# agsiddhant/PBML_Mantle_Convection

Measured on AMD Instinct MI355X. Metric: training samples/sec (2-D 506x506 Stokes fields), higher is better.
Workload: dtype f16+bf16; 1 GPU; CFG-3: symmetric U-Net (levels 5, c_h 16, k 5, repeats 3, reflect) + L1 data loss + divergence + Stokes momentum residual, 506x506, per-GPU batch 32, Adam, HIP-graph replay; global_batch=32, parallelism=dp1

## Files before the change

### include/mantle_hip.h

```cpp
#ifndef MANTLE_HIP_H
#define MANTLE_HIP_H

#include <stddef.h>
#include <stdint.h>

#ifdef __cplusplus
extern "C" {
#endif

#define MC_OK 0
#define MC_EINVAL (-1)
#define MC_EUNSUPPORTED (-2)
#define MC_EWORKSPACE (-3)

enum { MC_F32 = 0, MC_BF16 = 1, MC_MIX16 = 2 };
enum { MC_PAD_ZEROS = 0, MC_PAD_REPLICATE = 1, MC_PAD_REFLECT = 2 };
enum { MC_ACT_NONE = 0, MC_ACT_GELU = 1, MC_ACT_RELU = 2, MC_ACT_SILU = 3, MC_ACT_TANH = 4,
       MC_ACT_SELU = 5, MC_ACT_ELU = 6 };
enum { MC_POST_NONE = 0,
       MC_POST_ACT = 1,
       MC_POST_GN_ACT = 2   };
enum { MC_GSRC_NONE = 0,
       MC_GSRC_PLAIN = 1,
       MC_GSRC_PADFOLD = 2,
       MC_GSRC_PADFOLD_POOL = 3,
       MC_GSRC_PLAIN_POOL = 4   };

typedef struct {
  int32_t n;
  int32_t h, w;
  int32_t c_in0;
  int32_t c_in1;
  int32_t c_out;
  int32_t k;
  int32_t pad;
  int32_t pad_mode;
  int32_t dtype;
  int32_t sym_h;
  int32_t c_out_split;
  int32_t out_f32;
  int32_t sym_v;
  int32_t sym_hv;
} mc_conv_desc;

typedef struct {
  const void* ptr;
  int32_t kind;
  int32_t pad;
  int32_t pad_mode;
  int32_t pool;
  int32_t hs, ws;
  int32_t c8_total;
  int32_t cb_off;
} mc_grad_src;

typedef struct {
  const float* coef0;
  const float* coef1;
  int32_t act0, act1;
} mc_conv_prologue;

typedef struct {
  const void* y;
  const float* coef;
  int32_t act;
  int32_t pad;
  int32_t pad_mode;
  int32_t hs, ws;
  float* partials;
  int32_t part_stride;
  int32_t y_f16;
} mc_conv_epilogue;

int mc_version(void);
const char* mc_strerror(int code);

int mc_pack_nchw(const float* x, int32_t n, int32_t c, int32_t src_c, int32_t h, int32_t w, int32_t pad_w,
                 int32_t pad_mode, const float* chan_scale, int32_t dtype, void* out, void* stream);
int mc_unpack_nchw(const void* x, int32_t n, int32_t c, int32_t h, int32_t w, int32_t crop_w,
                   const float* mean_nc, int32_t dtype, float* out, void* stream);
int mc_pack_grad_nchw(const float* g, int32_t n, int32_t c, int32_t h, int32_t w, int32_t crop_w,
                      const float* mean_nc, int32_t dtype, void* out, void* stream);
int mc_sum_hw(const float* x, int32_t nc, int32_t hw, float scale, float* out, void* stream);

size_t mc_packed_weight_bytes(const mc_conv_desc* d, int32_t dgrad);
int mc_pack_weights(const mc_conv_desc* d, const float* w_unique, int32_t dgrad, void* packed,
                    void* stream);
const char* mc_conv_kernel_name(const mc_conv_desc* d);
int32_t mc_conv_tiles(const mc_conv_desc* d);
int mc_conv2d(const mc_conv_desc* d, const void* x0, const void* x1, const void* packed_w,
              const float* bias, void* y0, void* y1, float* stat_partials, void* stream);
int mc_conv2d_fused(const mc_conv_desc* d, const void* x0, const void* x1, const mc_conv_prologue* pro,
                    const void* packed_w, const float* bias, void* y0, void* y1, float* stat_partials,
                    const mc_conv_epilogue* epi, void* stream);
size_t mc_wgrad_partial_bytes(const mc_conv_desc* d);
size_t mc_conv_bank_read_extent(const mc_conv_desc* d);
int mc_conv2d_wgrad(const mc_conv_desc* d, const void* x0, const void* x1, const void* dy,
                    void* partials, void* stream);
int mc_conv2d_wgrad_finalize(const mc_conv_desc* d, const void* partials, float* dw_unique,
                             float* dbias, void* stream);
int mc_conv2d_wgrad_fused(const mc_conv_desc* d, const void* x0, const void* x1, const mc_conv_prologue* pro,
                          const void* dy, void* partials, void* stream);
int mc_pack_weights_batched(const mc_conv_desc* descs, const float* const* w_unique, const int32_t* dgrad,
                            void* const* packed, int32_t n, void* stream);
int mc_conv2d_wgrad_finalize_batched(const mc_conv_desc* descs, const void* const* partials, float* const* dw_unique,
                                     float* const* dbias, int32_t n, void* stream);

int mc_fold_padded(void* buf, int32_t n, int32_t c, int32_t hs, int32_t ws, int32_t pad, int32_t pad_mode,
                   int32_t dtype, void* stream);
int mc_fold_padded2(void* buf0, int32_t c0, void* buf1, int32_t c1, int32_t n, int32_t hs, int32_t ws, int32_t pad, int32_t pad_mode,
                    int32_t dtype, void* stream);
int32_t mc_fold_blocks(int32_t hs, int32_t ws, int32_t pad, int32_t pad_mode);
int mc_fold_padded_dz(void* buf, int32_t n, int32_t c, int32_t hs, int32_t ws, int32_t pad, int32_t pad_mode,
                      int32_t dtype, const void* y, const float* coef, int32_t act, float* partials,
                      int32_t part_stride_blocks, int32_t part_first_block, void* stream);

int mc_gn_partials(const void* y, int32_t n, int32_t c, int32_t h, int32_t w, int32_t dtype, int32_t tiles, float* part,
                   void* stream);
int mc_gn_finalize(const float* stat_partials, int32_t n, int32_t tiles, int32_t c, int32_t groups,
                   int32_t hw, float eps, float* stats_ng2, float* chan_mean, void* stream);
int mc_gn_finalize_coef(const float* stat_partials, int32_t n, int32_t tiles, int32_t c, int32_t groups, int32_t hw,
                        float eps, const float* gamma, const float* beta, float* stats_ng2, float* coef4, void* stream);

int mc_gn_act_fwd(const void* y, int32_t n, int32_t c, int32_t h, int32_t w, int32_t groups,
                  const float* stats_ng2, const float* gamma, const float* beta, int32_t post,
                  int32_t act, int32_t pool, int32_t dtype, void* a, void* pooled, void* stream);
int mc_gn_act_fwd_small(const void* y, const float* stat_partials, int32_t tiles, int32_t n, int32_t c, int32_t h, int32_t w,
                        int32_t groups, float eps, const float* gamma, const float* beta, int32_t act, int32_t pool,
                        int32_t dtype, float* stats_ng2, void* a, void* pooled, void* stream);
int32_t mc_gn_bwd_blocks(int32_t h, int32_t w);
int mc_gn_act_bwd_reduce(const void* y, int32_t n, int32_t c, int32_t h, int32_t w, int32_t groups,
                         const float* stats_ng2, const float* gamma, const float* beta, int32_t post,
                         int32_t act, int32_t dtype, const mc_grad_src* g0, const mc_grad_src* g1,
                         float* partials, void* stream);
int mc_gn_act_bwd_finalize(const float* partials, int32_t n, int32_t blocks, int32_t c, int32_t groups,
                           int32_t hw, const float* gamma, float* m12_ng2, float* dgamma, float* dbeta,
                           void* stream);
int mc_gn_act_bwd_finalize_n(const float* partials, int32_t n, int32_t blocks, int32_t c, int32_t groups, int32_t hw,
                             const float* gamma, float* m12_ng2, float* chan_sums, void* stream);
int mc_gn_act_bwd_apply(const void* y, int32_t n, int32_t c, int32_t h, int32_t w, int32_t groups,
                        const float* stats_ng2, const float* m12_ng2, const float* gamma,
                        const float* beta, int32_t post, int32_t act, int32_t dtype,
                        const mc_grad_src* g0, const mc_grad_src* g1, void* dy, void* stream);
int mc_gn_act_bwd_small(const void* y, int32_t n, int32_t c, int32_t h, int32_t w, int32_t groups, const float* stats_ng2,
                        const float* gamma, const float* beta, int32_t act, int32_t dtype, const mc_grad_src* g0,
                        const mc_grad_src* g1, void* dy, float* chan_sums, void* stream);
int mc_gn_param_grads_batched(const float* const* chan_sums, const int32_t* n, const int32_t* c, float* const* dgamma,
                              float* const* dbeta, int32_t jobs, void* stream);
int mc_gn_bwd_apply_dz(const mc_grad_src* dz, const void* y, int32_t n, int32_t c, int32_t h, int32_t w, int32_t groups,
                       const float* coef, const float* m12_ng2, int32_t dtype, void* dy, void* stream);
int mc_concat_cb8(const void* const* srcs, const int32_t* src_c, int32_t n_src, int32_t n, int32_t h, int32_t w,
                  int32_t dtype, void* out, void* stream);
int mc_cat_grad_gather(const mc_grad_src* g, int32_t c_total, int32_t c_off, int32_t c, int32_t n, int32_t h, int32_t w,
                       int32_t dtype, void* out, void* stream);
int mc_gsrc_sum(const mc_grad_src* g0, const mc_grad_src* g1, int32_t n, int32_t c, int32_t h, int32_t w,
                int32_t dtype, void* out, void* stream);

int mc_rect_copy(const void* src, int32_t hs, int32_t ws, int32_t sy, int32_t sx, void* dst, int32_t hd, int32_t wd,
                 int32_t dy, int32_t dx, int32_t rh, int32_t rw, int32_t n, int32_t c, int32_t accumulate, int32_t dtype,
                 void* stream);

int mc_avgpool_fwd(const void* x, int32_t n, int32_t c, int32_t h, int32_t w, int32_t f, int32_t dtype,
                   void* out, void* stream);
int mc_bicubic_fwd(const void* x, int32_t n, int32_t c, int32_t hi, int32_t wi, int32_t ho, int32_t wo,
                   const int32_t* idx_y, const float* wgt_y, const int32_t* idx_x, const float* wgt_x,
                   int32_t dtype, void* out, void* stream);
int mc_bicubic_fwd_act(const void* x, const float* coef, int32_t act, int32_t n, int32_t c, int32_t hi, int32_t wi,
                       int32_t ho, int32_t wo, const int32_t* idx_y, const float* wgt_y, const int32_t* idx_x,
                       const float* wgt_x, int32_t dtype, void* out, void* stream);
int mc_bicubic_bwd(const mc_grad_src* g, int32_t n, int32_t c, int32_t hi, int32_t wi, int32_t ho, int32_t wo,
                   const int32_t* ty_start, const int32_t* ty_j, const float* ty_w,
                   const int32_t* tx_start, const int32_t* tx_j, const float* tx_w,
                   int32_t dtype, void* dx, void* stream);
int mc_bicubic_bwd_taps(const mc_grad_src* gs, int32_t n, int32_t c, int32_t hi, int32_t wi, int32_t ho, int32_t wo,
                        const int32_t* tys, const int32_t* tyj, const float* tyw, const int32_t* txs, const int32_t* txj,
                        const float* txw, int32_t max_taps_y, int32_t max_taps_x, int32_t dtype, void* dx, void* stream);
int mc_bicubic_bwd_walk(const mc_grad_src* gs, int32_t n, int32_t c, int32_t hi, int32_t wi, int32_t ho, int32_t wo,
                        const int32_t* idx_y, const float* wgt_y, const int32_t* tys, const int32_t* tyj, const int32_t* txs,
                        const int32_t* txj, const float* txw, int32_t max_taps_x, int32_t dtype, void* dx, void* stream);
int mc_bicubic_bwd_separable(const mc_grad_src* g, int32_t n, int32_t c, int32_t hi, int32_t wi, int32_t ho, int32_t wo,
                             const int32_t* ty_start, const int32_t* ty_j, const float* ty_w,
                             const int32_t* tx_start, const int32_t* tx_j, const float* tx_w,
                             int32_t dtype, float* ws, void* dx, void* stream);

int mc_curl_head_fwd(const float* a, const float* t_in, int32_t n, int32_t h, int32_t w, int64_t in_batch_stride,
                     float a_bound, float t_lo, float t_hi, float* u, float* v, float* t_out, void* stream);
int mc_curl_head_bwd(const float* gu, const float* gv, const float* gt_out, const float* t_in, int32_t n, int32_t h,
                     int32_t w, float a_bound, float t_lo, float t_hi, float* ga, float* gt_in,
                     int64_t g_batch_stride, int64_t in_batch_stride, float* ws, void* stream);

int mc_curl_valid_fwd(const float* a, int32_t n, int32_t h, int32_t w, int64_t in_batch_stride, float a_bound, float* u,
                      float* v, void* stream);
int mc_curl_valid_bwd(const float* gu, const float* gv, int32_t n, int32_t h, int32_t w, float a_bound, float* ga,
                      int64_t g_batch_stride, void* stream);

#define MC_LOSS_SLOTS 16
enum { MC_S_U_SCALED = 0, MC_S_U_PLAIN, MC_S_V_SCALED, MC_S_V_PLAIN, MC_S_P_PLAIN, MC_S_T_PLAIN,
       MC_S_DU, MC_S_DV, MC_S_MASS, MC_S_MASS_X0, MC_S_MASS_X1, MC_S_MASS_Y0, MC_S_MASS_Y1,
       MC_S_MOMX, MC_S_MOMY, MC_S_SPARE };
typedef struct {
  int32_t n, h, w;
  int32_t p_pred;
  int32_t loss_type;
  int32_t loss_scale;
  int32_t loss_derivative;
  int32_t l2;
  float lambda_mom;
  float inv_h;
  float ra;
  int32_t t_grad;
} mc_loss_desc;
int mc_loss_minmax(const float* uvp, int32_t n, int32_t ct, int32_t h, int32_t w, float* mm, void* stream);
int mc_loss_fwd_bwd(const mc_loss_desc* d, const float* u, const float* v, const float* p, const float* T,
                    int64_t pred_batch_stride, int64_t p_batch_stride, const float* uvp, const float* mm,
                    double* sums, float* gu, float* gv, float* gp, float* gT, void* stream);
int mc_loss_fused(const mc_loss_desc* d, const float* u, const float* v, const float* p, const float* T, int64_t pbs, int64_t ppbs,
                  const float* y_cb8, int32_t cb8_w, int32_t cb8_crop, const float* cb8_mean, int32_t cb8_c, const float* uvp,
                  const float* mm, const float* yc, const float* paras, const float* scaler, double* sums, float* gu, float* gv,
                  float* gp, float* gT, int64_t g_pbs, int64_t g_ppbs, float* gsum_part, void* stream);
int32_t mc_loss_fused_blocks(int32_t n, int32_t h, int32_t w);
int mc_partial_sums_finalize(const float* part, int32_t n, int32_t blocks, int32_t c, float scale, float* out, void* stream);
int mc_momentum_residual(const mc_loss_desc* d, const float* u, const float* v, const float* p,
                         const float* T, int64_t pred_batch_stride, int64_t p_batch_stride, const float* yc, const float* paras,
                         const float* scaler, double* sums, float* sx, float* sy, float* eta_ws, void* stream);
int mc_momentum_adjoint(const mc_loss_desc* d, const float* T, int64_t pred_batch_stride, int64_t p_batch_stride, const float* eta_ws,
                        const float* paras, const float* scaler, const float* sx, const float* sy,
                        float* gu, float* gv, float* gp, float* gT, void* stream);
int mc_loss_finalize(const mc_loss_desc* d, const double* sums, float* out8, void* stream);

int mc_assemble_adtime_batch(const float* T, const float* uv, const float* t, const float* paras, const float* paras_nd,
                             const float* xc, const float* yc, const int32_t* pairs, int32_t b, int32_t m, int32_t cy,
                             int32_t h, int32_t w, float* x, float* y, float* scaler, float* paras_out, void* stream);

int mc_assemble_newad_batch(const float* T, const float* uvp, const float* t, const float* paras, const float* paras_nd,
                            const float* xc, const float* yc, const int32_t* idx, int32_t b, int32_t m, int32_t cy,
                            int32_t h, int32_t w, float* x, float* y, float* t_weight, float* scaler, void* stream);

int mc_roll_forward_update(float* x, int32_t c, const float* u, const float* v, const float* t, int64_t uvt_batch_stride,
                           const float* paras, int32_t update_v, int32_t n, int32_t h, int32_t w, void* stream);

int mc_ts_build_input(const float* T, const float* xc, const float* yc, const float* ycc, const float* paras,
                      const float* paras_nd, int32_t n, int32_t h, int32_t w, float* out, void* stream);
int mc_ts_build_input_unet(const float* T, const float* xc, const float* yc, const float* ycc, const float* paras,
                           const float* paras_nd, const float* dt, const float* u_prev, const float* v_prev, int32_t n,
                           int32_t h, int32_t w, float* out, void* stream);
int mc_ts_wall_bc(const float* t_in, int32_t n, int32_t h, int32_t w, float* t_out, void* stream);
int mc_adnet_step(const float* u, const float* v, int64_t uv_stride, const float* vel_scale, const float* T_prev,
                  const float* raq_field, const float* raq_scalar, const float* xc, const float* yc, int32_t n, int32_t h,
                  int32_t w, float cn_max, int32_t compute_dt, float* dt_io, uint32_t* ws, float* T_next, void* stream);

int mc_adam_step_flat(float* param, const float* grad, float* exp_avg, float* exp_avg_sq, int64_t numel,
                      const float* lr_dev, float beta1, float beta2, float eps, float weight_decay,
                      float grad_scale, int32_t* step_count_dev, void* stream);

#ifdef __cplusplus
}
#endif
#endif
```

### pbml_mantle_convection_amd/_lib.py

```python
import ctypes as C
import os

import torch

_HERE = os.path.dirname(os.path.abspath(__file__))
LIB_PATH = os.environ.get("MANTLE_LIB", os.path.join(_HERE, "libmantle_hip.so"))

MC_F32, MC_BF16, MC_MIX16 = 0, 1, 2
PAD_MODES = {"zeros": 0, "constant": 0, "replicate": 1, "reflect": 2}
ACTS = {"none": 0, "gelu": 1, "relu": 2, "silu": 3, "tanh": 4, "selu": 5, "elu": 6}
POST_NONE, POST_ACT, POST_GN_ACT = 0, 1, 2
GSRC_NONE, GSRC_PLAIN, GSRC_PADFOLD, GSRC_PADFOLD_POOL, GSRC_PLAIN_POOL = 0, 1, 2, 3, 4
LOSS_SLOTS = 16
LOSS_TYPES = {"mae": 0, "mass": 1, "curl": 2}


class ConvDesc(C.Structure):
    _fields_ = [(n, C.c_int32) for n in ("n", "h", "w", "c_in0", "c_in1", "c_out", "k", "pad", "pad_mode",
                                          "dtype", "sym_h", "c_out_split", "out_f32", "sym_v", "sym_hv")]


class GradSrc(C.Structure):
    _fields_ = [("ptr", C.c_void_p), ("kind", C.c_int32), ("pad", C.c_int32), ("pad_mode", C.c_int32),
                ("pool", C.c_int32), ("hs", C.c_int32), ("ws", C.c_int32), ("c8_total", C.c_int32), ("cb_off", C.c_int32)]


class ConvPrologue(C.Structure):
    _fields_ = [("coef0", C.c_void_p), ("coef1", C.c_void_p), ("act0", C.c_int32), ("act1", C.c_int32)]


class ConvEpilogue(C.Structure):
    _fields_ = [("y", C.c_void_p), ("coef", C.c_void_p), ("act", C.c_int32), ("pad", C.c_int32), ("pad_mode", C.c_int32),
                ("hs", C.c_int32), ("ws", C.c_int32), ("partials", C.c_void_p), ("part_stride", C.c_int32),
                ("y_f16", C.c_int32)]


class LossDesc(C.Structure):
    _fields_ = [("n", C.c_int32), ("h", C.c_int32), ("w", C.c_int32), ("p_pred", C.c_int32),
                ("loss_type", C.c_int32), ("loss_scale", C.c_int32), ("loss_derivative", C.c_int32),
                ("l2", C.c_int32), ("lambda_mom", C.c_float), ("inv_h", C.c_float), ("ra", C.c_float),
                ("t_grad", C.c_int32)]


_vp, _i32, _i64, _f32, _sz = C.c_void_p, C.c_int32, C.c_int64, C.c_float, C.c_size_t
_CD, _GS, _LD = C.POINTER(ConvDesc), C.POINTER(GradSrc), C.POINTER(LossDesc)
_CP, _CE = C.POINTER(ConvPrologue), C.POINTER(ConvEpilogue)

SIGNATURES = {
    "mc_version": (C.c_int, []),
    "mc_strerror": (C.c_char_p, [C.c_int]),
    "mc_pack_nchw": (C.c_int, [_vp, _i32, _i32, _i32, _i32, _i32, _i32, _i32, _vp, _i32, _vp, _vp]),
    "mc_unpack_nchw": (C.c_int, [_vp, _i32, _i32, _i32, _i32, _i32, _vp, _i32, _vp, _vp]),
    "mc_pack_grad_nchw": (C.c_int, [_vp, _i32, _i32, _i32, _i32, _i32, _vp, _i32, _vp, _vp]),
    "mc_sum_hw": (C.c_int, [_vp, _i32, _i32, _f32, _vp, _vp]),
    "mc_packed_weight_bytes": (_sz, [_CD, _i32]),
    "mc_conv_bank_read_extent": (_sz, [_CD]),
    "mc_pack_weights": (C.c_int, [_CD, _vp, _i32, _vp, _vp]),
    "mc_conv_tiles": (_i32, [_CD]),
    "mc_conv_kernel_name": (C.c_char_p, [_CD]),
    "mc_conv2d": (C.c_int, [_CD, _vp, _vp, _vp, _vp, _vp, _vp, _vp, _vp]),
    "mc_conv2d_fused": (C.c_int, [_CD, _vp, _vp, _CP, _vp, _vp, _vp, _vp, _vp, _CE, _vp]),
    "mc_conv2d_wgrad_fused": (C.c_int, [_CD, _vp, _vp, _CP, _vp, _vp, _vp]),
    "mc_gn_finalize_coef": (C.c_int, [_vp, _i32, _i32, _i32, _i32, _i32, _f32, _vp, _vp, _vp, _vp, _vp]),
    "mc_fold_blocks": (_i32, [_i32, _i32, _i32, _i32]),
    "mc_fold_padded_dz": (C.c_int, [_vp, _i32, _i32, _i32, _i32, _i32, _i32, _i32, _vp, _vp, _i32, _vp, _i32, _i32, _vp]),
    "mc_gn_bwd_apply_dz": (C.c_int, [_GS, _vp, _i32, _i32, _i32, _i32, _i32, _vp, _vp, _i32, _vp, _vp]),
    "mc_bicubic_fwd_act": (C.c_int, [_vp, _vp, _i32, _i32, _i32, _i32, _i32, _i32, _i32, _vp, _vp, _vp, _vp, _i32, _vp,
                                     _vp]),
    "mc_wgrad_partial_bytes": (_sz, [_CD]),
    "mc_conv2d_wgrad": (C.c_int, [_CD, _vp, _vp, _vp, _vp, _vp]),
    "mc_conv2d_wgrad_finalize": (C.c_int, [_CD, _vp, _vp, _vp, _vp]),
    "mc_pack_weights_batched": (C.c_int, [_CD, _vp, _vp, _vp, _i32, _vp]),
    "mc_conv2d_wgrad_finalize_batched": (C.c_int, [_CD, _vp, _vp, _vp, _i32, _vp]),
    "mc_fold_padded": (C.c_int, [_vp, _i32, _i32, _i32, _i32, _i32, _i32, _i32, _vp]),
    "mc_fold_padded2": (C.c_int, [_vp, _i32, _vp, _i32, _i32, _i32, _i32, _i32, _i32, _i32, _vp]),
    "mc_gn_partials": (C.c_int, [_vp, _i32, _i32, _i32, _i32, _i32, _i32, _vp, _vp]),
    "mc_gn_finalize": (C.c_int, [_vp, _i32, _i32, _i32, _i32, _i32, _f32, _vp, _vp, _vp]),
    "mc_gn_act_fwd": (C.c_int, [_vp, _i32, _i32, _i32, _i32, _i32, _vp, _vp, _vp, _i32, _i32, _i32, _i32, _vp,
                                _vp, _vp]),
    "mc_gn_bwd_blocks": (_i32, [_i32, _i32]),
    "mc_gn_act_bwd_reduce": (C.c_int, [_vp, _i32, _i32, _i32, _i32, _i32, _vp, _vp, _vp, _i32, _i32, _i32, _GS,
                                       _GS, _vp, _vp]),
    "mc_gn_act_bwd_finalize": (C.c_int, [_vp, _i32, _i32, _i32, _i32, _i32, _vp, _vp, _vp, _vp, _vp]),
    "mc_gn_act_bwd_finalize_n": (C.c_int, [_vp, _i32, _i32, _i32, _i32, _i32, _vp, _vp, _vp, _vp]),
    "mc_gn_act_bwd_apply": (C.c_int, [_vp, _i32, _i32, _i32, _i32, _i32, _vp, _vp, _vp, _vp, _i32, _i32, _i32,
                                      _GS, _GS, _vp, _vp]),
    "mc_gn_act_fwd_small": (C.c_int, [_vp, _vp, _i32, _i32, _i32, _i32, _i32, _i32, _f32, _vp, _vp, _i32, _i32, _i32, _vp, _vp, _vp,
                                      _vp]),
    "mc_gn_act_bwd_small": (C.c_int, [_vp, _i32, _i32, _i32, _i32, _i32, _vp, _vp, _vp, _i32, _i32, _GS, _GS, _vp, _vp, _vp]),
    "mc_gn_param_grads_batched": (C.c_int, [_vp, _vp, _vp, _vp, _vp, _i32, _vp]),
    "mc_avgpool_fwd": (C.c_int, [_vp, _i32, _i32, _i32, _i32, _i32, _i32, _vp, _vp]),
    "mc_rect_copy": (C.c_int, [_vp, _i32, _i32, _i32, _i32, _vp, _i32, _i32, _i32, _i32, _i32, _i32, _i32, _i32, _i32, _i32,
                               _vp]),
    "mc_concat_cb8": (C.c_int, [_vp, _vp, _i32, _i32, _i32, _i32, _i32, _vp, _vp]),
    "mc_gsrc_sum": (C.c_int, [_GS, _GS, _i32, _i32, _i32, _i32, _i32, _vp, _vp]),
    "mc_cat_grad_gather": (C.c_int, [_GS, _i32, _i32, _i32, _i32, _i32, _i32, _i32, _vp, _vp]),
    "mc_bicubic_fwd": (C.c_int, [_vp, _i32, _i32, _i32, _i32, _i32, _i32, _vp, _vp, _vp, _vp, _i32, _vp, _vp]),
    "mc_bicubic_bwd": (C.c_int, [_GS, _i32, _i32, _i32, _i32, _i32, _i32, _vp, _vp, _vp, _vp, _vp, _vp, _i32,
                                 _vp, _vp]),
    "mc_bicubic_bwd_walk": (C.c_int, [_GS, _i32, _i32, _i32, _i32, _i32, _i32, _vp, _vp, _vp, _vp, _vp, _vp, _vp, _i32, _i32, _vp, _vp]),
    "mc_bicubic_bwd_taps": (C.c_int, [_GS, _i32, _i32, _i32, _i32, _i32, _i32, _vp, _vp, _vp, _vp, _vp, _vp, _i32, _i32, _i32,
                                      _vp, _vp]),
    "mc_bicubic_bwd_separable": (C.c_int, [_GS, _i32, _i32, _i32, _i32, _i32, _i32, _vp, _vp, _vp, _vp, _vp, _vp, _i32,
                                           _vp, _vp, _vp]),
    "mc_curl_head_fwd": (C.c_int, [_vp, _vp, _i32, _i32, _i32, _i64, _f32, _f32, _f32, _vp, _vp, _vp, _vp]),
    "mc_curl_head_bwd": (C.c_int, [_vp, _vp, _vp, _vp, _i32, _i32, _i32, _f32, _f32, _f32, _vp, _vp, _i64, _i64,
                                   _vp, _vp]),
    "mc_curl_valid_fwd": (C.c_int, [_vp, _i32, _i32, _i32, _i64, _f32, _vp, _vp, _vp]),
    "mc_curl_valid_bwd": (C.c_int, [_vp, _vp, _i32, _i32, _i32, _f32, _vp, _i64, _vp]),
    "mc_assemble_adtime_batch": (C.c_int, [_vp, _vp, _vp, _vp, _vp, _vp, _vp, _vp, _i32, _i32, _i32, _i32, _i32, _vp, _vp,
                                           _vp, _vp, _vp]),
    "mc_assemble_newad_batch": (C.c_int, [_vp, _vp, _vp, _vp, _vp, _vp, _vp, _vp, _i32, _i32, _i32, _i32, _i32, _vp, _vp, _vp, _vp, _vp]),
    "mc_ts_build_input": (C.c_int, [_vp, _vp, _vp, _vp, _vp, _vp, _i32, _i32, _i32, _vp, _vp]),
    "mc_ts_build_input_unet": (C.c_int, [_vp, _vp, _vp, _vp, _vp, _vp, _vp, _vp, _vp, _i32, _i32, _i32, _vp, _vp]),
    "mc_roll_forward_update": (C.c_int, [_vp, _i32, _vp, _vp, _vp, _i64, _vp, _i32, _i32, _i32, _i32, _vp]),
    "mc_ts_wall_bc": (C.c_int, [_vp, _i32, _i32, _i32, _vp, _vp]),
    "mc_adnet_step": (C.c_int, [_vp, _vp, _i64, _vp, _vp, _vp, _vp, _vp, _vp, _i32, _i32, _i32, _f32, _i32, _vp, _vp, _vp,
                                _vp]),
    "mc_loss_minmax": (C.c_int, [_vp, _i32, _i32, _i32, _i32, _vp, _vp]),
    "mc_loss_fwd_bwd": (C.c_int, [_LD, _vp, _vp, _vp, _vp, _i64, _i64, _vp, _vp, _vp, _vp, _vp, _vp, _vp, _vp]),
    "mc_loss_fused": (C.c_int, [_LD, _vp, _vp, _vp, _vp, _i64, _i64, _vp, _i32, _i32, _vp, _i32, _vp, _vp, _vp, _vp, _vp, _vp, _vp, _vp,
                                _vp, _vp, _i64, _i64, _vp, _vp]),
    "mc_loss_fused_blocks": (_i32, [_i32, _i32, _i32]),
    "mc_partial_sums_finalize": (C.c_int, [_vp, _i32, _i32, _i32, _f32, _vp, _vp]),
    "mc_momentum_residual": (C.c_int, [_LD, _vp, _vp, _vp, _vp, _i64, _i64, _vp, _vp, _vp, _vp, _vp, _vp, _vp, _vp]),
    "mc_momentum_adjoint": (C.c_int, [_LD, _vp, _i64, _i64, _vp, _vp, _vp, _vp, _vp, _vp, _vp, _vp, _vp, _vp]),
    "mc_loss_finalize": (C.c_int, [_LD, _vp, _vp, _vp]),
    "mc_adam_step_flat": (C.c_int, [_vp, _vp, _vp, _vp, _i64, _vp, _f32, _f32, _f32, _f32, _f32, _vp, _vp]),
}

VALUE_RETURNING = {"mc_version", "mc_strerror", "mc_conv_kernel_name", "mc_packed_weight_bytes", "mc_conv_bank_read_extent", "mc_conv_tiles",
                   "mc_wgrad_partial_bytes", "mc_gn_bwd_blocks", "mc_fold_blocks", "mc_loss_fused_blocks"}

_lib = None


def load():
    global _lib
    if _lib is not None:
        return _lib
    if not os.path.exists(LIB_PATH):
        raise RuntimeError(
            f"{LIB_PATH} is missing: build it with `python -m pbml_mantle_convection_amd.build_ext` "
            "(hipcc --offload-arch=gfx950).  There is no CPU fallback for the hot path.")
    lib = C.CDLL(LIB_PATH)
    for name, (res, args) in SIGNATURES.items():
        fn = getattr(lib, name)
        fn.restype = res
        fn.argtypes = args
    _lib = lib
    return lib


class MantleHipError(RuntimeError):
    pass


def check(rc, what=""):
    if rc != 0:
        msg = load().mc_strerror(int(rc)).decode()
        raise MantleHipError(f"libmantle_hip: {what} failed with code {rc}: {msg}")


def ptr(t):
    if t is None:
        return None
    return t.data_ptr()


def stream():
    return torch.cuda.current_stream().cuda_stream


def call(name, *args):
    fn = getattr(load(), name)
    rc = fn(*args)
    if name not in VALUE_RETURNING:
        check(rc, name)
    return rc


def require_cuda(t, name="tensor"):
    if not isinstance(t, torch.Tensor) or not t.is_cuda:
        raise RuntimeError(
            f"{name} must live on the MI355X (HIP device tensor): this framework's hot path is HIP-only and "
            "has no CPU fallback")
```

### pbml_mantle_convection_amd/csrc/conv_api.hip

```cpp
#include "conv_rr.h"

int mc_conv2d_f32(const ConvGeom& g, const void* x0, const void* x1, const void* bank, const float* bias, void* y0,
                  void* y1, float* part, const ConvFuse& fz, int fuse, hipStream_t s);
int mc_wgrad_f32(const ConvGeom& g, const void* x0, const void* x1, const void* dy, void* part, const ConvFuse& fz, int fuse,
                 hipStream_t s);
int mc_bf16_tile(const mc_conv_desc* d, int* th, int* tw);
size_t mc_bf16_bank_bytes(const ConvGeom& g, int dgrad);
int mc_bf16_pack(const ConvGeom& g, const float* w_unique, int dgrad, void* packed, hipStream_t s);
int mc_conv2d_bf16(const ConvGeom& g, const void* x0, const void* x1, const void* bank, const float* bias, void* y0,
                   void* y1, float* part, const ConvFuse& fz, int fuse, hipStream_t s);
int mc_wgrad_bf16(const ConvGeom& g, const void* x0, const void* x1, const void* dy, void* part, const ConvFuse& fz, int fuse,
                  hipStream_t s);
const char* mc_bf16_kernel_name(const ConvGeom& g);
void mc_bf16_bank_dims(const ConvGeom& g, int dgrad, int& chunks, int& steps, int& ntiles);
bool mc_rr_applies(int dtype, int cout, int wo, bool full_pad);
size_t mc_rr_bank_bytes(const ConvGeom& g, int dgrad);
int mc_rr_pack(const ConvGeom& g, const float* w_unique, int dgrad, void* packed, hipStream_t s);
int mc_conv2d_rr(const ConvGeom& g, const void* x0, const void* x1, const void* bank, const float* bias, void* y0, void* y1,
                 float* part, const ConvFuse& fz, int fuse, hipStream_t s);
const char* mc_rr_kernel_name(const ConvGeom& g, int fuse);

namespace {

bool rr_desc(const mc_conv_desc* d) {
  return mc_rr_applies(d->dtype, d->c_out, d->w + 2 * d->pad - d->k + 1, d->pad == d->k - 1);
}

int geom_for(const mc_conv_desc* d, ConvGeom& g) {
  if (!d) return MC_EINVAL;
  int th = 16, tw = 16;
  if (mc_is16(d->dtype)) {
    if (rr_desc(d)) { th = RR_R; tw = RR_TW; }
    else {
      int rc = mc_bf16_tile(d, &th, &tw);
      if (rc) return rc;
    }
  } else if (d->dtype != MC_F32) {
    return MC_EUNSUPPORTED;
  }
  return conv_geom(d, th, tw, g);
}
int stat_slots(const mc_conv_desc* d, const ConvGeom& g) { return rr_desc(d) ? g.tiles * RR_STRIPS : g.tiles; }

__global__ void k_pack_f32(ConvGeom g, const float* __restrict__ wu, int dgrad, float* __restrict__ bank, size_t total) {
  for (size_t i = blockIdx.x * (size_t)blockDim.x + threadIdx.x; i < total; i += (size_t)gridDim.x * blockDim.x)
    bank[i] = pack_value_f32(g, wu, i, dgrad);
}

struct PkJob {
  int K, Cout, CBin, CB0, Cin0, Cin1, Cin, U, nh, nv, nq, CBout, CinP, CoutP;
  int dgrad, steps, ntiles, bf16, f16, rr, first_block;
  unsigned total;
  const float* w;
  void* out;
};
constexpr int PK_MAX = 24;
struct PkTable { int n; PkJob j[PK_MAX]; };

__global__ void k_pack_batched(PkTable t) {
  int ji = 0;
#pragma unroll 1
  for (int k = 1; k < t.n; ++k) if ((int)blockIdx.x >= t.j[k].first_block) ji = k;
  const PkJob& job = t.j[ji];
  const int nblk = (ji + 1 < t.n ? t.j[ji + 1].first_block : (int)gridDim.x) - job.first_block;
  for (size_t i = (size_t)(blockIdx.x - job.first_block) * blockDim.x + threadIdx.x; i < job.total; i += (size_t)nblk * blockDim.x) {
    if (job.rr || job.bf16) {
      const float v = job.rr ? rr_pack_value(job, job.w, i, job.dgrad, job.ntiles)
                             : pack_value_bf16(job, job.w, i, job.dgrad, job.steps, job.ntiles);
      reinterpret_cast<bf16_t*>(job.out)[i] = job.f16 ? __builtin_bit_cast(bf16_t, (_Float16)v) : f2bf(v);
    } else {
      reinterpret_cast<float*>(job.out)[i] = pack_value_f32(job, job.w, i, job.dgrad);
    }
  }
}

struct WfJob {
  int K, U, nh, nv, nq, Cin, Cin0, CB0, CinP, CoutP, Cout, G, first_block;
  const float* part;
  float* dw;
  float* db;
};
constexpr int WF_MAX = 32;
struct WfTable { int n; WfJob j[WF_MAX]; };

constexpr int WF_WAVES = 16;
__device__ __forceinline__ void wgrad_finalize_block(const WfJob& g, int lblock) {
  const int K = g.K, KK = K * K;
  const int nch = wg_chunks(g.CinP);
  const size_t slab = wg_slab_floats(g.CoutP, g.CinP, KK);
  const size_t nW = (size_t)KK * nch * g.U * 16;
  const size_t total = nW + g.Cout;
  const int e = threadIdx.x & 63, w = threadIdx.x >> 6, NWV = (int)blockDim.x >> 6;
  const size_t i = (size_t)lblock * 64 + e;
  __shared__ float red[WF_WAVES][64];
  float s = 0.f;
  long dst = -1;
  if (i < total) {
    size_t o1, ox[3] = {0, 0, 0};
    int nx = 0;
    bool live = true;
    if (i < nW) {
      int cl = (int)(i & 15);
      size_t r = i >> 4;
      int u = (int)(r % g.U); r /= g.U;
      int chunk = (int)(r % nch);
      int tap = (int)(r / nch);
      int cip = chunk * 16 + cl;
      int ci = cip < g.CB0 * 8 ? cip : g.Cin0 + (cip - g.CB0 * 8);
      live = cip < g.CB0 * 8 ? cip < g.Cin0 : ci < g.Cin;
      int ky = tap / K, kx = tap - ky * K;
      o1 = wg_index(tap, cip, u, g.CoutP, nch);
      const int tfx = ky * K + (K - 1 - kx), tfy = (K - 1 - ky) * K + kx, tfxy = (K - 1 - ky) * K + (K - 1 - kx);
      if (u < g.nh) { nx = 1; ox[0] = wg_index(tfx, cip, g.U + u, g.CoutP, nch); }
      else if (u < g.nh + g.nv) { nx = 1; ox[0] = wg_index(tfy, cip, g.U + u, g.CoutP, nch); }
      else if (u < g.nh + g.nv + g.nq) {
        const int c0 = g.U + g.nh + g.nv + (u - g.nh - g.nv);
        nx = 3;
        ox[0] = wg_index(tfx, cip, c0, g.CoutP, nch); ox[1] = wg_index(tfy, cip, c0 + g.nq, g.CoutP, nch);
        ox[2] = wg_index(tfxy, cip, c0 + 2 * g.nq, g.CoutP, nch);
      }
      dst = ((long)u * g.Cin + ci) * KK + tap;
    } else {
      o1 = (size_t)KK * nch * g.CoutP * 16 + (i - nW);
      dst = -2 - (long)(i - nW);
    }
    if (live) {
      const float* part = g.part;
      float a0 = 0.f, a1 = 0.f, a2 = 0.f, a3 = 0.f;
      int G = w;
      for (; G + 3 * NWV < g.G; G += 4 * NWV) {
        a0 += part[(size_t)G * slab + o1]; a1 += part[(size_t)(G + NWV) * slab + o1];
        a2 += part[(size_t)(G + 2 * NWV) * slab + o1]; a3 += part[(size_t)(G + 3 * NWV) * slab + o1];
        for (int m = 0; m < nx; ++m) {
          a0 += part[(size_t)G * slab + ox[m]]; a1 += part[(size_t)(G + NWV) * slab + ox[m]];
          a2 += part[(size_t)(G + 2 * NWV) * slab + ox[m]]; a3 += part[(size_t)(G + 3 * NWV) * slab + ox[m]];
        }
      }
      for (; G < g.G; G += NWV) {
        a0 += part[(size_t)G * slab + o1];
        for (int m = 0; m < nx; ++m) a0 += part[(size_t)G * slab + ox[m]];
      }
      s = (a0 + a1) + (a2 + a3);
    } else {
      dst = -1;
    }
  }
  red[w][e] = s;
  __syncthreads();
  if (w == 0 && dst != -1) {
    float r = 0.f;
    for (int k = 0; k < NWV; k += 4) r += (red[k][e] + red[k + 1][e]) + (red[k + 2][e] + red[k + 3][e]);
    if (dst >= 0) { if (g.dw) g.dw[dst] += r; }
    else if (g.db) g.db[-2 - dst] += r;
  }
}

__global__ __launch_bounds__(64 * WF_WAVES) void k_wgrad_finalize(WfTable t) {
  int ji = 0;
#pragma unroll 1
  for (int k = 1; k < t.n; ++k) if ((int)blockIdx.x >= t.j[k].first_block) ji = k;
  wgrad_finalize_block(t.j[ji], blockIdx.x - t.j[ji].first_block);
}

int wf_fill(const mc_conv_desc* d, const void* partials, float* dw, float* db, WfJob& j, int& blocks) {
  ConvGeom g;
  int rc = geom_for(d, g);
  if (rc) return rc;
  if (!partials || (!dw && !db)) return MC_EINVAL;
  j.K = g.K; j.U = g.U; j.Cin = g.Cin; j.Cin0 = g.Cin0; j.CB0 = g.CB0; j.CinP = g.CinP; j.CoutP = g.CoutP; j.Cout = g.Cout;
  j.nh = g.nh; j.nv = g.nv; j.nq = g.nq; j.G = g.wgrad_G; j.part = (const float*)partials; j.dw = dw; j.db = db;
  size_t total = (size_t)g.K * g.K * wg_chunks(g.CinP) * g.U * 16 + g.Cout;
  blocks = (int)((total + 63) / 64);
  return MC_OK;
}

}

static bool bank_is_rr(const ConvGeom& g, int dgrad) {
  return dgrad ? mc_rr_applies(g.dtype, g.Cin, g.W + 2 * g.pad, true) : mc_rr_applies(g.dtype, g.Cout, g.Wo, g.pad == g.K - 1);
}

extern "C" {

int mc_version(void) { return 200; }

const char* mc_strerror(int code) {
  switch (code) {
    case MC_OK: return "ok";
    case MC_EINVAL: return "invalid argument or shape";
    case MC_EUNSUPPORTED: return "unsupported configuration";
    case MC_EWORKSPACE: return "workspace too small";
    default: return code > 0 ? hipGetErrorString((hipError_t)code) : "unknown error";
  }
}

size_t mc_packed_weight_bytes(const mc_conv_desc* d, int32_t dgrad) {
  ConvGeom g;
  if (geom_for(d, g)) return 0;
  if (bank_is_rr(g, dgrad)) return mc_rr_bank_bytes(g, dgrad);
  if (mc_is16(g.dtype)) return mc_bf16_bank_bytes(g, dgrad);
  int cbin = dgrad ? g.CBout : g.CBin, cop = dgrad ? g.CinP : g.CoutP;
  return (size_t)cbin * g.K * g.K * 8 * cop * sizeof(float);
}

int mc_pack_weights(const mc_conv_desc* d, const float* w_unique, int32_t dgrad, void* packed, void* stream) {
  ConvGeom g;
  int rc = geom_for(d, g);
  if (rc) return rc;
  if (!w_unique || !packed) return MC_EINVAL;
  if (bank_is_rr(g, dgrad)) return mc_rr_pack(g, w_unique, dgrad, packed, (hipStream_t)stream);
  if (mc_is16(g.dtype)) return mc_bf16_pack(g, w_unique, dgrad, packed, (hipStream_t)stream);
  size_t total = mc_packed_weight_bytes(d, dgrad) / sizeof(float);
  int blocks = (int)((total + 255) / 256);
  if (blocks > 2048) blocks = 2048;
  hipLaunchKernelGGL(k_pack_f32, dim3(blocks), dim3(256), 0, (hipStream_t)stream, g, w_unique, dgrad, (float*)packed, total);
  MC_CHECK_LAUNCH();
  return MC_OK;
}

const char* mc_conv_kernel_name(const mc_conv_desc* d) {
  ConvGeom g;
  if (geom_for(d, g)) return "unsupported";
  if (rr_desc(d)) return mc_rr_kernel_name(g, 0);
  if (mc_is16(g.dtype)) return mc_bf16_kernel_name(g);
  return g.K == 5 ? "k_conv_direct_f32<5>" : "k_conv_direct_f32<3>";
}

int32_t mc_conv_tiles(const mc_conv_desc* d) {
  ConvGeom g;
  if (geom_for(d, g)) return -1;
  return stat_slots(d, g);
}

static bool act_ok(int a) { return a >= MC_ACT_NONE && a <= MC_ACT_ELU; }

static int fill_prologue(const mc_conv_prologue* pro, ConvFuse& fz, int& rc) {
  rc = MC_OK;
  if (!pro) return 0;
  if (!act_ok(pro->act0) || !act_ok(pro->act1)) { rc = MC_EINVAL; return 0; }
  fz.coef0 = pro->coef0; fz.coef1 = pro->coef1; fz.act0 = pro->act0; fz.act1 = pro->act1;
  return (pro->coef0 || pro->coef1 || pro->act0 != MC_ACT_NONE || pro->act1 != MC_ACT_NONE) ? 1 : 0;
}

int mc_conv2d_fused(const mc_conv_desc* d, const void* x0, const void* x1, const mc_conv_prologue* pro,
                    const void* packed_w, const float* bias, void* y0, void* y1, float* stat_partials,
                    const mc_conv_epilogue* epi, void* stream) {
  ConvGeom g;
  int rc = geom_for(d, g);
  if (rc) return rc;
  if (!x0 || !packed_w || !y0 || (g.Cin1 > 0 && !x1) || (g.split8 > 0 && !y1)) return MC_EINVAL;
  ConvFuse fz = conv_fuse_none();
  int fuse = fill_prologue(pro, fz, rc);
  if (rc) return rc;
  if (epi) {
    if (fuse) return MC_EUNSUPPORTED;
    if (!epi->y || !epi->partials || !act_ok(epi->act) || epi->pad < 0 || epi->hs <= 0 || epi->ws <= 0) return MC_EINVAL;
    if (epi->pad_mode < MC_PAD_ZEROS || epi->pad_mode > MC_PAD_REFLECT) return MC_EINVAL;
    if (g.split8 > 0 || stat_partials || g.out_f32) return MC_EUNSUPPORTED;
    if (g.Ho != epi->hs + 2 * epi->pad || g.Wo != epi->ws + 2 * epi->pad) return MC_EINVAL;
    fz.ey = epi->y; fz.ecoef = epi->coef; fz.epart = epi->partials; fz.eact = epi->act; fz.epad = epi->pad;
    fz.ezero = epi->pad_mode == MC_PAD_ZEROS || epi->pad == 0; fz.ehs = epi->hs; fz.ews = epi->ws;
    if (epi->y_f16 && g.dtype != MC_BF16) return MC_EINVAL;
    fz.ey16 = epi->y_f16 ? 1 : 0;
    if (epi->part_stride < stat_slots(d, g)) return MC_EINVAL;
    fz.estride = epi->part_stride;
    fuse = 2;
  }
  if (rr_desc(d)) return mc_conv2d_rr(g, x0, x1, packed_w, bias, y0, y1, stat_partials, fz, fuse, (hipStream_t)stream);
  if (mc_is16(g.dtype)) return mc_conv2d_bf16(g, x0, x1, packed_w, bias, y0, y1, stat_partials, fz, fuse, (hipStream_t)stream);
  return mc_conv2d_f32(g, x0, x1, packed_w, bias, y0, y1, stat_partials, fz, fuse, (hipStream_t)stream);
}

int mc_conv2d(const mc_conv_desc* d, const void* x0, const void* x1, const void* packed_w, const float* bias, void* y0,
              void* y1, float* stat_partials, void* stream) {
  return mc_conv2d_fused(d, x0, x1, nullptr, packed_w, bias, y0, y1, stat_partials, nullptr, stream);
}

size_t mc_conv_bank_read_extent(const mc_conv_desc* d) {
  ConvGeom g;
  if (geom_for(d, g)) return 0;
  const int KK = g.K * g.K;
  if (rr_desc(d)) {
    const size_t nfrag = g.K == 5 ? RR<5>::NFRAG : RR<3>::NFRAG;
    const size_t chunks = (g.CBin + 1) / 2, groups = (g.Cout + 15) / 16;
    return (((chunks - 1) * groups + (groups - 1)) * nfrag * 64 + (nfrag * 64 - 1)) * 16 + 16;
  }
  if (mc_is16(g.dtype)) {
    int chunks, steps, ntiles;
    mc_bf16_bank_dims(g, 0, chunks, steps, ntiles);
    const size_t last = ((size_t)(chunks - 1) * steps + (steps - 1)) * ntiles + (ntiles - 1);
    return (last * 64 + 63) * 16 + 16;
  }
  const int ncog = (g.CoutP + 15) / 16, co0 = 16 * (ncog - 1);
  const int comax = g.CoutP - 1 - co0;
  const size_t last = (((size_t)(g.CBin - 1) * KK + (KK - 1)) * 8 + 7) * g.CoutP + co0 + (comax >= 15 ? 15 : comax);
  return (last + 1) * sizeof(float);
}

size_t mc_wgrad_partial_bytes(const mc_conv_desc* d) {
  ConvGeom g;
  if (geom_for(d, g)) return 0;
  return (size_t)g.wgrad_G * wg_slab_floats(g.CoutP, g.CinP, g.K * g.K) * sizeof(float);
}

int mc_conv2d_wgrad_fused(const mc_conv_desc* d, const void* x0, const void* x1, const mc_conv_prologue* pro,
                          const void* dy, void* partials, void* stream) {
  ConvGeom g;
  int rc = geom_for(d, g);
  if (rc) return rc;
  if (!x0 || !dy || !partials || (g.Cin1 > 0 && !x1)) return MC_EINVAL;
  ConvFuse fz = conv_fuse_none();
  const int fuse = fill_prologue(pro, fz, rc);
  if (rc) return rc;
  if (mc_is16(g.dtype)) return mc_wgrad_bf16(g, x0, x1, dy, partials, fz, fuse, (hipStream_t)stream);
  return mc_wgrad_f32(g, x0, x1, dy, partials, fz, fuse, (hipStream_t)stream);
}

int mc_conv2d_wgrad(const mc_conv_desc* d, const void* x0, const void* x1, const void* dy, void* partials,
                    void* stream) {
  return mc_conv2d_wgrad_fused(d, x0, x1, nullptr, dy, partials, stream);
}

int mc_conv2d_wgrad_finalize_batched(const mc_conv_desc* descs, const void* const* partials, float* const* dw,
                                     float* const* db, int32_t n, void* stream) {
  if (!descs || !partials || !dw || !db || n <= 0) return MC_EINVAL;
  for (int pass = 0; pass < 2; ++pass) {
    WfTable t;
    t.n = 0;
    int blocks = 0;
    auto flush = [&]() {
      if (t.n == 0) return;
      hipLaunchKernelGGL(k_wgrad_finalize, dim3(blocks), dim3(pass == 0 ? 64 * WF_WAVES : 256), 0, (hipStream_t)stream, t);
      t.n = 0; blocks = 0;
    };
    for (int k = 0; k < n; ++k) {
      WfJob j;
      int b = 0;
      int rc = wf_fill(&descs[k], partials[k], dw[k], db[k], j, b);
      if (rc) return rc;
      if ((j.G >= 128) != (pass == 0)) continue;
      j.first_block = blocks;
      t.j[t.n++] = j;
      blocks += b;
      if (t.n == WF_MAX) flush();
    }
    flush();
    MC_CHECK_LAUNCH();
  }
  return MC_OK;
}

int mc_conv2d_wgrad_finalize(const mc_conv_desc* d, const void* partials, float* dw_unique, float* dbias,
                             void* stream) {
  return mc_conv2d_wgrad_finalize_batched(d, &partials, &dw_unique, &dbias, 1, stream);
}

int mc_pack_weights_batched(const mc_conv_desc* descs, const float* const* w_unique, const int32_t* dgrad,
                            void* const* packed, int32_t n, void* stream) {
  if (!descs || !w_unique || !dgrad || !packed || n <= 0) return MC_EINVAL;
  for (int base = 0; base < n; base += PK_MAX) {
    PkTable t;
    t.n = n - base < PK_MAX ? n - base : PK_MAX;
    int blocks = 0;
    for (int k = 0; k < t.n; ++k) {
      ConvGeom g;
      int rc = geom_for(&descs[base + k], g);
      if (rc) return rc;
      if (!w_unique[base + k] || !packed[base + k]) return MC_EINVAL;
      PkJob& j = t.j[k];
      j.K = g.K; j.Cout = g.Cout; j.CBin = g.CBin; j.CB0 = g.CB0; j.Cin0 = g.Cin0; j.Cin1 = g.Cin1; j.Cin = g.Cin; j.U = g.U;
      j.nh = g.nh; j.nv = g.nv; j.nq = g.nq;
      j.CBout = g.CBout; j.CinP = g.CinP; j.CoutP = g.CoutP; j.dgrad = dgrad[base + k]; j.bf16 = mc_is16(g.dtype);
      j.f16 = (g.dtype == MC_MIX16 && !j.dgrad) ? 1 : 0;
      j.rr = bank_is_rr(g, j.dgrad);
      size_t total;
      if (j.rr) {
        j.steps = 0;
        j.ntiles = ((j.dgrad ? g.CinP : g.Cout) + 15) / 16;
        total = mc_rr_bank_bytes(g, j.dgrad) / 2;
      } else if (j.bf16) {
        int chunks;
        mc_bf16_bank_dims(g, j.dgrad, chunks, j.steps, j.ntiles);
        total = (size_t)chunks * j.steps * j.ntiles * 64 * 8;
      } else {
        j.steps = 0; j.ntiles = 0;
        total = (size_t)(j.dgrad ? g.CBout : g.CBin) * g.K * g.K * 8 * (j.dgrad ? g.CinP : g.CoutP);
      }
      j.total = (unsigned)total;
      j.w = w_unique[base + k];
      j.out = packed[base + k];
      j.first_block = blocks;
      int b = (int)((total + 256 * 8 - 1) / (256 * 8));
      blocks += b < 1 ? 1 : b;
    }
    hipLaunchKernelGGL(k_pack_batched, dim3(blocks), dim3(256), 0, (hipStream_t)stream, t);
    MC_CHECK_LAUNCH();
  }
  return MC_OK;
}

}
```

### pbml_mantle_convection_amd/csrc/conv_bf16.hip

```cpp
#include "conv_common.h"
#include <type_traits>

using bf16x8 = __attribute__((ext_vector_type(8))) short;
using f16x8 = __attribute__((ext_vector_type(8))) _Float16;
using f32x4 = __attribute__((ext_vector_type(4))) float;
typedef unsigned int v4u __attribute__((ext_vector_type(4)));

namespace {

__device__ __forceinline__ int xcd_remap(int bid, int nwg) {
  const int xcd = bid & 7, q = nwg >> 3, r = nwg & 7;
  return (xcd < r ? xcd * (q + 1) : r * (q + 1) + (xcd - r) * q) + (bid >> 3);
}

constexpr int CHUNK_CB = 2;

template <int K> struct KSteps { static constexpr int pairs = K * K * CHUNK_CB; static constexpr int steps = (pairs + 3) / 4; };

struct Bf16Cfg { int th, tw, nt, mt; };

__host__ __device__ inline int pick_nt(int n_tiles) { return (n_tiles % 4 == 0) ? 4 : ((n_tiles % 2 == 0) ? 2 : 1); }

__global__ void k_pack_bf16(ConvGeom g, const float* __restrict__ wu, int dgrad, bf16_t* __restrict__ bank,
                            int chunks, int steps, int ntiles, int f16) {
  const size_t total = (size_t)chunks * steps * ntiles * 64 * 8;
  for (size_t i = blockIdx.x * (size_t)blockDim.x + threadIdx.x; i < total; i += (size_t)gridDim.x * blockDim.x) {
    const float v = pack_value_bf16(g, wu, i, dgrad, steps, ntiles);
    bank[i] = f16 ? __builtin_bit_cast(bf16_t, (_Float16)v) : f2bf(v);
  }
}

template <bool H16> __device__ __forceinline__ f32x4 mfma16(bf16x8 a, bf16x8 b, f32x4 c) {
  if constexpr (H16) return __builtin_amdgcn_mfma_f32_16x16x32_f16(__builtin_bit_cast(f16x8, a), __builtin_bit_cast(f16x8, b), c, 0, 0, 0);
  else return __builtin_amdgcn_mfma_f32_16x16x32_bf16(a, b, c, 0, 0, 0);
}

#ifdef MC_EXP_NOSYNC
#define MC_SYNC() do {} while (0)
#else
#define MC_SYNC() __syncthreads()
#endif
template <int K, int TH, int TW, int NT, int MT, bool OUT_F32 = false, int FUSE = 0, bool H16 = false, int WN = 1>
#ifndef MC_CONV_WAVES
#define MC_CONV_WAVES 2
#endif
__global__ __launch_bounds__(64 * (TH * (TW / 16) / MT) * WN, (MT * NT / WN <= 8 ? MC_CONV_WAVES : 2)) void k_conv_mfma_bf16(
    ConvGeom g, const bf16_t* __restrict__ x0, const bf16_t* __restrict__ x1, const bf16_t* __restrict__ bank,
    const float* __restrict__ bias, bf16_t* __restrict__ y0, bf16_t* __restrict__ y1, float* __restrict__ part,
    int n_groups, ConvFuse fz) {
  constexpr int TIH = TH + K - 1, TIW = TW + K - 1;
  constexpr int PLANE = (TIH * TIW + 15) / 16 * 16;
  constexpr int STEPS = KSteps<K>::steps;
  constexpr int MTILES_X = TW / 16;
  constexpr int WAVES = TH * MTILES_X / MT * WN, NTHR = 64 * WAVES;
  constexpr int NTW = NT / WN;
  static_assert(TH * MTILES_X * WN == WAVES * MT && NTW * WN == NT && (WAVES == 4 || WAVES == 8), "tile / wave decomposition mismatch");
  constexpr int IN_SLOTS = CHUNK_CB * PLANE;
#ifndef MC_WGLOBAL_ALL
#define MC_WGLOBAL_ALL 0
#endif
  constexpr bool WGLOBAL = NT > 1 || MC_WGLOBAL_ALL;
  constexpr int W_SLOTS = WGLOBAL ? 0 : STEPS * NT * 64;
  static_assert(!OUT_F32 || NT == 1, "f32 output is for the single-N-tile configuration");
  constexpr int IN_ELEMS = CHUNK_CB * TIH * TIW;
  constexpr int IN_ITERS = (IN_ELEMS + NTHR - 1) / NTHR;
  constexpr int W_ITERS = WGLOBAL ? 1 : (W_SLOTS + NTHR - 1) / NTHR;
  __shared__ uint4 lds[IN_SLOTS + (WGLOBAL ? 1 : W_SLOTS)];
  __shared__ float red[WAVES][NT * 16 * 2];
  uint4* in_s = lds;
  uint4* w_s = lds + IN_SLOTS;

  const int grp = blockIdx.y;
  const int bid = xcd_remap(blockIdx.x, gridDim.x);
  const int lane = threadIdx.x & 63, wave = __builtin_amdgcn_readfirstlane(threadIdx.x >> 6);
  const int m = lane & 15, gq = lane >> 4;
  const int ntile0 = grp * NT;
  const int wm = wave / WN, nt_w0 = (wave % WN) * NTW;
  const int ntiles_total = gridDim.y * NT;
  const int chunks = (g.CBin + CHUNK_CB - 1) / CHUNK_CB;
  const int items = g.N * g.tiles;
  const int my_items = (items - bid + (int)gridDim.x - 1) / (int)gridDim.x;
  const int total_stages = my_items * chunks;

  constexpr int PER_CB = (TIH * TIW + NTHR - 1) / NTHR;
  static_assert(IN_ITERS <= CHUNK_CB * PER_CB, "");
  v4u rin[CHUNK_CB][PER_CB];
  float psc[CHUNK_CB][8], psh[CHUNK_CB][8];
  int pact[CHUNK_CB] = {-1, -1};
  unsigned okm = 0xffffffffu;
  int s_rc[PER_CB];
  unsigned s_off[PER_CB];
  int s_lds[PER_CB];
#pragma unroll
  for (int it = 0; it < PER_CB; ++it) {
    int i = threadIdx.x + it * NTHR;
    bool live = i < TIH * TIW;
    if (!live) i = TIH * TIW - 1;
    int r = i / TIW, c = i - r * TIW;
    s_rc[it] = (live ? 0 : (1 << 31)) | (r << 15) | c;
    s_off[it] = (unsigned)(r * g.W + c) * 16u;
    s_lds[it] = live ? r * TIW + c : -1;
  }
  auto prefetch = [&](int t) {
    const int jitem = t / chunks, ck = t - jitem * chunks;
    const int wi = bid + jitem * (int)gridDim.x;
    const int n = wi / g.tiles, tile = wi - n * g.tiles;
    const int ty0 = (tile / g.tiles_x) * TH, tx0 = (tile % g.tiles_x) * TW;
    const bool interior = (ty0 - g.pad >= 0) && (ty0 - g.pad + TIH <= g.H) && (tx0 - g.pad >= 0) && (tx0 - g.pad + TIW <= g.W);
    const unsigned org16 = (unsigned)((ty0 - g.pad) * g.W + (tx0 - g.pad)) * 16u;
#pragma unroll
    for (int cb = 0; cb < CHUNK_CB; ++cb) {
      const int gcb = ck * CHUNK_CB + cb;
      const int gcc = min(gcb, g.CBin - 1);
      const bool second = gcc >= g.CB0;
      const int scb = second ? gcc - g.CB0 : gcc;
      const int sC8 = second ? g.CB1 : g.CB0;
      const size_t plane_bytes = (size_t)g.H * g.W * 16;
      const char* pbase = reinterpret_cast<const char*>(second ? x1 : x0) + ((size_t)n * sC8 + scb) * plane_bytes;
      __amdgpu_buffer_rsrc_t rs = __builtin_amdgcn_make_buffer_rsrc((void*)pbase, 0, gcb < g.CBin ? (int)plane_bytes : 0, 0x00020000);
      if constexpr (FUSE == 1) {
        const float* ct = second ? fz.coef1 : fz.coef0;
        const int a = second ? fz.act1 : fz.act0;
        pact[cb] = (gcb < g.CBin && (ct != nullptr || a != MC_ACT_NONE)) ? a : -1;
        if (pact[cb] >= 0) load_coef8(ct, n, sC8 * 8, scb, psc[cb], psh[cb]);
        if (cb == 0) okm = 0xffffffffu;
      }
#pragma unroll
      for (int it = 0; it < PER_CB; ++it) {
        unsigned off;
        if (interior) {
          off = org16 + s_off[it];
        } else {
          int r = (s_rc[it] >> 15) & 0x7fff, c = s_rc[it] & 0x7fff;
          bool oky, okx;
          int sy = pad_map_sel(ty0 + r - g.pad, g.H, g.pad_mode, oky);
          int sx = pad_map_sel(tx0 + c - g.pad, g.W, g.pad_mode, okx);
          off = (oky && okx) ? (unsigned)(sy * g.W + sx) * 16u : 0xFFFFFFF0u;
          if (FUSE == 1 && cb == 0 && !(oky && okx)) okm &= ~(1u << it);
        }
#ifdef MC_EXP_NOLOAD
        rin[cb][it] = (v4u){off, off, off, off};
#else
        rin[cb][it] = __builtin_amdgcn_raw_buffer_load_b128(rs, off, 0, 0);
#endif
      }
    }
  };
  auto commit = [&]() {
#pragma unroll
    for (int cb = 0; cb < CHUNK_CB; ++cb) {
      if (FUSE == 1 && pact[cb] >= 0) {
#pragma unroll
        for (int it = 0; it < PER_CB; ++it)
          if (s_lds[it] >= 0) {
            const uint4 raw = make_uint4(rin[cb][it][0], rin[cb][it][1], rin[cb][it][2], rin[cb][it][3]);
            uint4 v = H16 ? xform_f16x8(raw, psc[cb], psh[cb], pact[cb]) : xform_bf16x8(raw, psc[cb], psh[cb], pact[cb]);
            if (!((okm >> it) & 1u)) v = make_uint4(0, 0, 0, 0);
            in_s[cb * PLANE + s_lds[it]] = v;
          }
        continue;
      }
#pragma unroll
      for (int it = 0; it < PER_CB; ++it)
        if (s_lds[it] >= 0)
          in_s[cb * PLANE + s_lds[it]] = make_uint4(rin[cb][it][0], rin[cb][it][1], rin[cb][it][2], rin[cb][it][3]);
    }
  };
  auto stage_weights = [&](int ck) {
    const uint4* bsrc = reinterpret_cast<const uint4*>(bank) + (size_t)ck * STEPS * ntiles_total * 64;
    uint4 rw[W_ITERS];
#pragma unroll
    for (int it = 0; it < W_ITERS; ++it) {
      int i = min((int)threadIdx.x + it * NTHR, W_SLOTS - 1);
      int ln = i & 63;
      int r = i >> 6;
      int tt = r % NT, ss = r / NT;
      rw[it] = bsrc[((size_t)ss * ntiles_total + ntile0 + tt) * 64 + ln];
    }
#pragma unroll
    for (int it = 0; it < W_ITERS; ++it) {
      int i = threadIdx.x + it * NTHR;
      if (i < W_SLOTS) w_s[i] = rw[it];
    }
  };

  float bv[NTW][4];
#pragma unroll
  for (int tt = 0; tt < NTW; ++tt)
#pragma unroll
    for (int r = 0; r < 4; ++r) {
      int co = (ntile0 + nt_w0 + tt) * 16 + gq * 4 + r;
      bv[tt][r] = (bias && co < g.Cout) ? bias[co] : 0.f;
    }

#ifndef MC_PREFETCH_ALL
#define MC_PREFETCH_ALL 0
#endif
  constexpr bool PREFETCH = (NT == 1) || MC_PREFETCH_ALL;
  f32x4 acc[MT][NTW];
  if (PREFETCH && total_stages > 0) prefetch(0);
#ifdef MC_EXP_STAMPS
  long long st_acc[7] = {0, 0, 0, 0, 0, 0, 0};
#define STAMP(k) do { long long now_ = clock64(); st_acc[k] += now_ - st_prev; st_prev = now_; } while (0)
#else
#define STAMP(k) do {} while (0)
#endif
  for (int t = 0; t < total_stages; ++t) {
#ifdef MC_EXP_STAMPS
    long long st_prev = clock64();
#endif
    const int jitem = t / chunks, ck = t - jitem * chunks;
    if (ck == 0) {
#pragma unroll
      for (int i = 0; i < MT; ++i)
#pragma unroll
        for (int tt = 0; tt < NTW; ++tt) acc[i][tt] = (f32x4){bv[tt][0], bv[tt][1], bv[tt][2], bv[tt][3]};
    }
    if (!PREFETCH) prefetch(t);
    MC_SYNC();
    STAMP(0);
    commit();
    if (!WGLOBAL && (chunks > 1 || t == 0)) stage_weights(ck);
    const uint4* wglob = reinterpret_cast<const uint4*>(bank) + ((size_t)ck * STEPS * ntiles_total + ntile0 + nt_w0) * 64 + lane;
    STAMP(1);
    MC_SYNC();
    STAMP(2);
    if (PREFETCH && t + 1 < total_stages) prefetch(t + 1);
    STAMP(3);
    const int wbase = (wm * MT / MTILES_X) * TIW + ((wm * MT) % MTILES_X) * 16 + m;
    int kx = gq >> 1, ky = 0;
    const int cbk_off = (gq & 1) * PLANE + wbase;
    auto load_frags = [&](int sidx, bf16x8 (&xf)[MT], bf16x8 (&wf)[NTW]) {
      const bool dummy = ky >= K;
      const uint4* ap = in_s + (cbk_off + (dummy ? 0 : ky * TIW + kx));
      kx += 2;
      if (kx >= K) { kx -= K; ky += 1; }
#pragma unroll
      for (int tt = 0; tt < NTW; ++tt) {
        if (WGLOBAL) {
#ifdef MC_EXP_NOWLOAD
          uint4 wv = make_uint4(sidx, tt, lane, 0);
#else
          uint4 wv = wglob[((size_t)sidx * ntiles_total + tt) * 64];
#endif
          wf[tt] = __builtin_bit_cast(bf16x8, wv);
        } else {
          wf[tt] = *reinterpret_cast<const bf16x8*>(&w_s[(sidx * NT + tt) * 64 + lane]);
        }
      }
#pragma unroll
      for (int i = 0; i < MT; ++i)
        xf[i] = *reinterpret_cast<const bf16x8*>(ap + (i / MTILES_X) * TIW + (i % MTILES_X) * 16);
    };
    auto do_mfma = [&](const bf16x8 (&xf)[MT], const bf16x8 (&wf)[NTW]) {
#pragma unroll
      for (int i = 0; i < MT; ++i)
#pragma unroll
        for (int tt = 0; tt < NTW; ++tt) acc[i][tt] = mfma16<(H16 && FUSE != 2)>(wf[tt], xf[i], acc[i][tt]);
    };
#ifndef MC_KPIPE
#define MC_KPIPE 0
#endif
#ifndef MC_KUNROLL
#define MC_KUNROLL 1
#endif
    if constexpr (WGLOBAL && MC_KUNROLL) {
#ifndef MC_KDEPTH
#define MC_KDEPTH 2
#endif
    constexpr int KD = MC_KDEPTH;
    bf16x8 xr[KD][MT], wr[KD][NTW];
#pragma unroll
    for (int s = 0; s < KD - 1 && s < STEPS; ++s) load_frags(s, xr[s], wr[s]);
#pragma unroll
    for (int s = 0; s < STEPS; ++s) {
      if (s + KD - 1 < STEPS) load_frags(s + KD - 1, xr[(s + KD - 1) % KD], wr[(s + KD - 1) % KD]);
      __builtin_amdgcn_sched_barrier(0);
      do_mfma(xr[s % KD], wr[s % KD]);
      __builtin_amdgcn_sched_barrier(0);
    }
    } else if constexpr (WGLOBAL || MC_KPIPE == 2) {
    bf16x8 xa[MT], xb[MT], wa[NTW], wb[NTW];
    load_frags(0, xa, wa);
#pragma unroll 1
    for (int s = 0; s < STEPS; s += 2) {
      if (s + 1 < STEPS) load_frags(s + 1, xb, wb);
      do_mfma(xa, wa);
      if (s + 2 < STEPS) load_frags(s + 2, xa, wa);
      if (s + 1 < STEPS) do_mfma(xb, wb);
    }
    } else {
    bf16x8 xa[MT], wa[NTW];
#pragma unroll 1
#ifdef MC_EXP_NOK
    for (int s = 0; s < 1; ++s) {
#else
    for (int s = 0; s < STEPS; ++s) {
#endif
      load_frags(s, xa, wa);
#if MC_KPIPE == 1
      __builtin_amdgcn_sched_group_barrier(0x100, MT + NTW, 0);
#endif
      do_mfma(xa, wa);
#if MC_KPIPE == 1
      __builtin_amdgcn_sched_group_barrier(0x008, MT * NTW, 0);
#endif
    }
    }
    STAMP(4);
    if (ck != chunks - 1) continue;

    const int wi = bid + jitem * (int)gridDim.x;
    const int n = wi / g.tiles, tile = wi - n * g.tiles;
    const int ty0 = (tile / g.tiles_x) * TH, tx0 = (tile % g.tiles_x) * TW;
    f32x2 s1[NTW][2], s2[NTW][2];
#pragma unroll
    for (int tt = 0; tt < NTW; ++tt)
#pragma unroll
      for (int h = 0; h < 2; ++h) { s1[tt][h] = (f32x2){0.f, 0.f}; s2[tt][h] = (f32x2){0.f, 0.f}; }
    const int oy0 = ty0 + (wm * MT) / MTILES_X, ox0 = tx0 + ((wm * MT) % MTILES_X) * 16 + m;
    char* dst0[NTW];
    bool cobok[NTW];
#pragma unroll
    for (int tt = 0; tt < NTW; ++tt) {
      const int cob = (ntile0 + nt_w0 + tt) * 2 + (gq >> 1);
      cobok[tt] = cob < g.CBout;
      const int cbc = min(cob, g.CBout - 1);
      const int esz = OUT_F32 ? 4 : 2;
      if (g.split8 > 0 && cbc >= g.split8)
        dst0[tt] = reinterpret_cast<char*>(y1) + (cb8_index(n, cbc - g.split8, oy0, ox0, g.CBout - g.split8, g.Ho, g.Wo) + (gq & 1) * 4) * esz;
      else
        dst0[tt] = reinterpret_cast<char*>(y0) + (cb8_index(n, cbc, oy0, ox0, g.split8 > 0 ? g.split8 : g.CBout, g.Ho, g.Wo) + (gq & 1) * 4) * esz;
    }
    const size_t row_bytes = (size_t)g.Wo * 8 * (OUT_F32 ? 4 : 2);
    auto emit = [&](auto full_tag) {
      constexpr bool FULL = decltype(full_tag)::value;
#pragma unroll
      for (int i = 0; i < MT; ++i) {
        const int oy = oy0 + i / MTILES_X, ox = ox0 + (i % MTILES_X) * 16;
        const bool inb = FULL || (oy < g.Ho && ox < g.Wo);
        const size_t off = (size_t)(i / MTILES_X) * row_bytes + (size_t)(i % MTILES_X) * 16 * 8 * (OUT_F32 ? 4 : 2);
#pragma unroll
        for (int tt = 0; tt < NTW; ++tt) {
          const f32x2 v01 = (f32x2){acc[i][tt][0], acc[i][tt][1]}, v23 = (f32x2){acc[i][tt][2], acc[i][tt][3]};
          if (inb) {
            s1[tt][0] += v01; s1[tt][1] += v23;
            s2[tt][0] = pk_fma(v01, v01, s2[tt][0]); s2[tt][1] = pk_fma(v23, v23, s2[tt][1]);
          }
#ifdef MC_EXP_NOSTORE
          if (inb && cobok[tt] && v01.x == 123.456f) {
#else
          if (inb && cobok[tt]) {
#endif
            if (OUT_F32) {
              *reinterpret_cast<float4*>(dst0[tt] + off) = make_float4(v01.x, v01.y, v23.x, v23.y);
            } else {
              uint2 pk;
              if constexpr (H16) { pk.x = pk_f16(v01.x, v01.y); pk.y = pk_f16(v23.x, v23.y); }
              else { pk.x = pk_bf16(v01.x, v01.y); pk.y = pk_bf16(v23.x, v23.y); }
              *reinterpret_cast<uint2*>(dst0[tt] + off) = pk;
            }
          }
        }
      }
    };
    auto emit_dz = [&]() {
      const int p = fz.epad, fr = fz.ezero ? 0 : p + 1;
      const int CBe = g.CBout;
      const bf16_t* ey = reinterpret_cast<const bf16_t*>(fz.ey);
#pragma unroll
      for (int tt = 0; tt < NTW; ++tt) {
        const int cob = (ntile0 + nt_w0 + tt) * 2 + (gq >> 1);
        const int cbc = min(cob, g.CBout - 1);
        float csc[4], csh[4], cme[4], crs[4];
#pragma unroll
        for (int r = 0; r < 4; ++r) {
          if (fz.ecoef) {
            const float4 c4 = reinterpret_cast<const float4*>(fz.ecoef)[(size_t)n * g.CoutP + cbc * 8 + (gq & 1) * 4 + r];
            csc[r] = c4.x; csh[r] = c4.y; cme[r] = c4.z; crs[r] = c4.w;
          } else { csc[r] = 1.f; csh[r] = 0.f; cme[r] = 0.f; crs[r] = 0.f; }
        }
        uint2 yv[MT];
        bool fin[MT];
#pragma unroll
        for (int i = 0; i < MT; ++i) {
          const int iy = oy0 + i / MTILES_X - p, ix = ox0 + (i % MTILES_X) * 16 - p;
          fin[i] = cobok[tt] && iy >= fr && iy < fz.ehs - fr && ix >= fr && ix < fz.ews - fr;
          const int cy = min(max(iy, 0), fz.ehs - 1), cx = min(max(ix, 0), fz.ews - 1);
          yv[i] = *reinterpret_cast<const uint2*>(ey + cb8_index(n, cbc, cy, cx, CBe, fz.ehs, fz.ews) + (gq & 1) * 4);
        }
#pragma unroll
        for (int i = 0; i < MT; ++i) {
          const int oy = oy0 + i / MTILES_X, ox = ox0 + (i % MTILES_X) * 16;
          const bool inb = oy < g.Ho && ox < g.Wo;
          const size_t off = (size_t)(i / MTILES_X) * row_bytes + (size_t)(i % MTILES_X) * 16 * 8 * 2;
          float yf[4];
          if constexpr (H16) {
            const f32x2 ya = unpk_f16(yv[i].x), yb = unpk_f16(yv[i].y);
            yf[0] = ya.x; yf[1] = ya.y; yf[2] = yb.x; yf[3] = yb.y;
          } else {
            yf[0] = __uint_as_float(yv[i].x << 16); yf[1] = __uint_as_float(yv[i].x & 0xffff0000u);
            yf[2] = __uint_as_float(yv[i].y << 16); yf[3] = __uint_as_float(yv[i].y & 0xffff0000u);
          }
          float o[4];
#pragma unroll
          for (int h = 0; h < 2; ++h) {
            const f32x2 yy = (f32x2){yf[2 * h], yf[2 * h + 1]};
            const f32x2 z = pk_fma(yy, (f32x2){csc[2 * h], csc[2 * h + 1]}, (f32x2){csh[2 * h], csh[2 * h + 1]});
            f32x2 gp;
            if (fz.eact == MC_ACT_GELU) gp = gelu_grad_poly2(z);
            else gp = (f32x2){act_bwd(z.x, fz.eact), act_bwd(z.y, fz.eact)};
            const f32x2 da = (f32x2){acc[i][tt][2 * h], acc[i][tt][2 * h + 1]};
            const f32x2 dz = da * gp;
            const f32x2 yh = (yy - (f32x2){cme[2 * h], cme[2 * h + 1]}) * (f32x2){crs[2 * h], crs[2 * h + 1]};
            if (fin[i]) { s1[tt][h] += dz; s2[tt][h] = pk_fma(dz, yh, s2[tt][h]); }
            o[2 * h] = fin[i] ? dz.x : da.x; o[2 * h + 1] = fin[i] ? dz.y : da.y;
          }
          if (inb && cobok[tt]) {
            uint2 pk;
            pk.x = (uint32_t)f2bf(o[0]) | ((uint32_t)f2bf(o[1]) << 16);
            pk.y = (uint32_t)f2bf(o[2]) | ((uint32_t)f2bf(o[3]) << 16);
            *reinterpret_cast<uint2*>(dst0[tt] + off) = pk;
          }
        }
      }
    };
    if constexpr (FUSE == 2) emit_dz();
    else { if (ty0 + TH <= g.Ho && tx0 + TW <= g.Wo) emit(std::true_type{}); else emit(std::false_type{}); }
    STAMP(5);
    if (FUSE == 2) part = fz.epart;
    if (part) {
#pragma unroll
      for (int tt = 0; tt < NTW; ++tt) {
        float q8[8] = {s1[tt][0].x, s2[tt][0].x, s1[tt][0].y, s2[tt][0].y, s1[tt][1].x, s2[tt][1].x, s1[tt][1].y, s2[tt][1].y};
        const bool b3 = m & 8, b2 = m & 4, b1 = m & 2;
        float q4[4], q2[2], q1;
#pragma unroll
        for (int k = 0; k < 4; ++k) q4[k] = (b3 ? q8[4 + k] : q8[k]) + __shfl_xor(b3 ? q8[k] : q8[4 + k], 8, 64);
#pragma unroll
        for (int k = 0; k < 2; ++k) q2[k] = (b2 ? q4[2 + k] : q4[k]) + __shfl_xor(b2 ? q4[k] : q4[2 + k], 4, 64);
        q1 = (b1 ? q2[1] : q2[0]) + __shfl_xor(b1 ? q2[0] : q2[1], 2, 64);
        q1 += __shfl_xor(q1, 1, 64);
        if ((m & 1) == 0) red[wave][((nt_w0 + tt) * 16 + gq * 4) * 2 + (m >> 1)] = q1;
      }
      MC_SYNC();
      if (threadIdx.x < NT * 32) {
        int co = ntile0 * 16 + (threadIdx.x >> 1);
        if (co < g.CoutP) {
          float r = 0.f;
#pragma unroll
          for (int wv = 0; wv < WAVES / WN; ++wv) r += red[wv * WN + (int)(threadIdx.x >> 5) / NTW][threadIdx.x];
          part[(((size_t)n * (FUSE == 2 ? fz.estride : g.tiles) + tile) * g.CoutP + co) * 2 + (threadIdx.x & 1)] = r;
        }
      }
    }
    STAMP(6);
  }
#ifdef MC_EXP_STAMPS
  if (blockIdx.x == 777 && blockIdx.y == 0 && threadIdx.x == 0)
    printf("stamps tiles %d: wait1 %lld commit %lld wait2 %lld pfetch %lld kloop %lld epi %lld stats %lld\n", my_items, st_acc[0], st_acc[1], st_acc[2], st_acc[3], st_acc[4], st_acc[5], st_acc[6]);
#endif
}

typedef short v4s __attribute__((ext_vector_type(4)));
typedef __attribute__((address_space(3))) v4s lds_v4s;

__device__ __forceinline__ bf16x8 tr_frag(const short* base_lo) {
  v4s lo = __builtin_amdgcn_ds_read_tr16_b64_v4i16((lds_v4s*)base_lo);
  v4s hi = __builtin_amdgcn_ds_read_tr16_b64_v4i16((lds_v4s*)(base_lo + 32));
  return (bf16x8){lo[0], lo[1], lo[2], lo[3], hi[0], hi[1], hi[2], hi[3]};
}

constexpr int WTH = 16, WTW = 32;
#ifndef MC_WGRAD_BATCH_NTW
#define MC_WGRAD_BATCH_NTW 1
#endif

template <int K, int NTW, int RS, bool PRO = false, bool XH = false>
__global__ __launch_bounds__(256, (NTW == 1 && RS >= 2) ? 3 : 2) void k_wgrad_mfma_bf16(ConvGeom g, const bf16_t* __restrict__ x0,
                                                            const bf16_t* __restrict__ x1, const bf16_t* __restrict__ dy,
                                                            float* __restrict__ part, int tiles_x, int tiles, ConvFuse fz) {
  static_assert(RS == 0 || RS == 1 || RS == 2 || RS == 4, "tap groups");
  constexpr int NS = RS ? RS : 1;
  constexpr int NG = 4 / NS;
  constexpr int TPW = (K * K + NS) / NS;
  constexpr int KK = K * K;
  constexpr int TIH = WTH + K - 1, TIW = WTW + K - 1;
  constexpr int XRS = RS ? (TIW + 11) / 16 * 16 + 4 : TIW;
  constexpr int DRS = RS ? WTW + 4 : WTW;
  constexpr int XPS = RS ? (TIH * XRS + 15) / 16 * 16 + 8 : ((TIH * TIW + 15) / 16) * 16 + 4;
  constexpr int DPS = RS ? WTH * DRS + 8 : WTH * WTW + 4;
  static_assert(!RS || (XRS >= TIW && XRS >= 3 * 8 + 12 && XRS % 16 == 4 && DRS % 16 == 4 && XPS % 16 == 8 && DPS % 16 == 8),
                "register-shift LDS layout");
  constexpr int NTAP = (KK + 3) / 4;
  constexpr int NACC = RS ? TPW * NTW : NTAP * NTW;
  constexpr int X_ITERS = (TIH * TIW + 255) / 256;
  constexpr int D_ELEMS = NTW * 2 * WTH * WTW, D_ITERS = D_ELEMS / 256;
  static_assert(D_ELEMS % 256 == 0, "dy tile must divide evenly over the threads");
  __shared__ uint4 smem[2 * XPS + NTW * 2 * DPS];
  static_assert(RS == 0 || RS == 4 || sizeof(smem) >= NS * NACC * 256 * sizeof(float), "cross-wave reduction reuses the tile buffers");
  uint4* const xs = smem;
  uint4* const ds = smem + 2 * XPS;
  const int chunk = blockIdx.y, cog = blockIdx.z;
  const int bid = xcd_remap(blockIdx.x, gridDim.x);
  const int lane = threadIdx.x & 63, wave = __builtin_amdgcn_readfirstlane(threadIdx.x >> 6);
  const int q = (lane & 15) >> 2, p = lane & 3, gq = lane >> 4;
  const int tg = wave % NS, cg = wave / NS;
  const int col0 = 8 * NS * cg;
  const int lane_x = RS ? ((p >> 1) * XPS + gq * XRS + col0 + q) * 8 + (p & 1) * 4 : ((p >> 1) * XPS + 8 * gq + q) * 8 + (p & 1) * 4;
  const int lane_d = RS ? ((p >> 1) * DPS + gq * DRS + col0 + q) * 8 + (p & 1) * 4 : ((p >> 1) * DPS + 8 * gq + q) * 8 + (p & 1) * 4;
  const short* xs_s = reinterpret_cast<const short*>(xs);
  const short* ds_s = reinterpret_cast<const short*>(ds);
  static_assert(3 + 4 * (NTAP - 1) >= KK, "wave 3 needs a free accumulator slot for the bias gradient");
  const bool do_bias = (RS == 0 ? wave == 3 : tg == NS - 1) && (chunk == 0);
  const bf16x8 ones = (bf16x8){0x3F80, 0x3F80, 0x3F80, 0x3F80, 0x3F80, 0x3F80, 0x3F80, 0x3F80};
  const ptrdiff_t x1_delta = x1 ? reinterpret_cast<const char*>(x1) - reinterpret_cast<const char*>(x0) : (ptrdiff_t)0;

  int toff[NTAP];
#pragma unroll
  for (int ti = 0; ti < NTAP; ++ti) {
    int tap = wave + 4 * ti;
    toff[ti] = tap < KK ? ((tap / K) * TIW + (tap % K)) * 8 : -1;
  }
  const short* xtap[NTAP];
#pragma unroll
  for (int ti = 0; ti < NTAP; ++ti) xtap[ti] = xs_s + lane_x + max(toff[ti], 0);
  int x_rc[X_ITERS];
  unsigned x_off[X_ITERS];
#pragma unroll
  for (int it = 0; it < X_ITERS; ++it) {
    int i = threadIdx.x + it * 256;
    bool live = i < TIH * TIW;
    if (!live) i = TIH * TIW - 1;
    int r = i / TIW, c = i - r * TIW;
    x_rc[it] = (live ? 0 : (1 << 31)) | (r << 15) | c;
    x_off[it] = (unsigned)(r * g.W + c) * 16u;
  }
  static_assert(WTW == 32 && WTH == 16, "dy staging decode");
  const int d_r0 = threadIdx.x >> 5, d_c0 = threadIdx.x & 31;
  const unsigned d_off0 = (unsigned)(d_r0 * g.Wo + d_c0) * 16u;
  const int d_lds0 = d_r0 * DRS + d_c0;
  const bool co_full = (cog * NTW + NTW) * 2 <= g.CBout;
  const char* xbase[2];
  bool xok[2];
  int xC8[2];
#pragma unroll
  for (int cb = 0; cb < 2; ++cb) {
    int gcb = chunk * 2 + cb;
    xok[cb] = gcb < g.CBin;
    int gcc = min(gcb, g.CBin - 1);
    bool second = gcc >= g.CB0;
    xC8[cb] = second ? g.CB1 : g.CB0;
    xbase[cb] = reinterpret_cast<const char*>(x0) + (second ? x1_delta : (ptrdiff_t)0) +
                cb8_index(0, second ? gcc - g.CB0 : gcc, 0, 0, xC8[cb], g.H, g.W) * sizeof(bf16_t);
  }

  uint4 rx[2][X_ITERS], rd[D_ITERS];
  float psc[2][8], psh[2][8];
  int pact[2] = {-1, -1};
  unsigned okm = 0xffffffffu;
  auto prefetch = [&](int wi_fwd) __attribute__((always_inline)) {
    const int wi = wi_fwd;
    const int n = wi / tiles, tile = wi - n * tiles;
    const int ty0 = (tile / tiles_x) * WTH, tx0 = (tile % tiles_x) * WTW;
    const bool interior = (ty0 - g.pad >= 0) && (ty0 - g.pad + TIH <= g.H) && (tx0 - g.pad >= 0) && (tx0 - g.pad + TIW <= g.W);
    const char* bpn[2] = {xbase[0] + (size_t)n * xC8[0] * g.H * g.W * 16, xbase[1] + (size_t)n * xC8[1] * g.H * g.W * 16};
    if constexpr (PRO) {
#pragma unroll
      for (int cb = 0; cb < 2; ++cb) {
        const int gcb = min(chunk * 2 + cb, g.CBin - 1);
        const bool second = gcb >= g.CB0;
        const float* ct = second ? fz.coef1 : fz.coef0;
        const int a = second ? fz.act1 : fz.act0;
        pact[cb] = (xok[cb] && (ct != nullptr || a != MC_ACT_NONE)) ? a : -1;
        if (pact[cb] >= 0) load_coef8(ct, n, xC8[cb] * 8, second ? gcb - g.CB0 : gcb, psc[cb], psh[cb]);
      }
      okm = 0xffffffffu;
    }
    if (interior) {
      const size_t org = (size_t)((ty0 - g.pad) * g.W + (tx0 - g.pad)) * 16;
#pragma unroll
      for (int cb = 0; cb < 2; ++cb)
#pragma unroll
        for (int it = 0; it < X_ITERS; ++it) {
          uint4 v = *reinterpret_cast<const uint4*>(bpn[cb] + org + x_off[it]);
          rx[cb][it] = xok[cb] ? v : make_uint4(0, 0, 0, 0);
        }
    } else {
#pragma unroll
      for (int it = 0; it < X_ITERS; ++it) {
        int r = (x_rc[it] >> 15) & 0x7fff, c = x_rc[it] & 0x7fff;
        bool oky, okx;
        int sy = pad_map_sel(ty0 + r - g.pad, g.H, g.pad_mode, oky);
        int sx = pad_map_sel(tx0 + c - g.pad, g.W, g.pad_mode, okx);
        const bool ok = oky && okx;
        if (PRO && !ok) okm &= ~(1u << it);
#pragma unroll
        for (int cb = 0; cb < 2; ++cb) {
          uint4 v = *reinterpret_cast<const uint4*>(bpn[cb] + (size_t)(sy * g.W + sx) * 16);
          rx[cb][it] = (ok && xok[cb]) ? v : make_uint4(0, 0, 0, 0);
        }
      }
    }
    if (co_full && ty0 + WTH <= g.Ho && tx0 + WTW <= g.Wo) {
      const char* db = reinterpret_cast<const char*>(dy) + cb8_index(n, cog * NTW * 2, ty0, tx0, g.CBout, g.Ho, g.Wo) * sizeof(bf16_t);
#pragma unroll
      for (int it = 0; it < D_ITERS; ++it)
        rd[it] = *reinterpret_cast<const uint4*>(db + (size_t)((it >> 1) * g.Ho + 8 * (it & 1)) * g.Wo * 16 + d_off0);
      return;
    }
#pragma unroll
    for (int it = 0; it < D_ITERS; ++it) {
      int i = threadIdx.x + it * 256;
      int pl = i / (WTH * WTW);
      int rem = i - pl * (WTH * WTW);
      int r = rem / WTW, c = rem - r * WTW;
      int cob = (cog * NTW) * 2 + pl;
      int oy = ty0 + r, ox = tx0 + c;
      bool ok = cob < g.CBout && oy < g.Ho && ox < g.Wo;
      uint4 v = *reinterpret_cast<const uint4*>(dy + cb8_index(n, min(cob, g.CBout - 1), min(oy, g.Ho - 1), min(ox, g.Wo - 1),
                                                               g.CBout, g.Ho, g.Wo));
      rd[it] = ok ? v : make_uint4(0, 0, 0, 0);
    }
  };
  auto commit = [&]() __attribute__((always_inline)) {
#pragma unroll
    for (int cb = 0; cb < 2; ++cb)
#pragma unroll
      for (int it = 0; it < X_ITERS; ++it)
      {
        int v = x_rc[it];
        asm volatile("" : "+v"(v));
        if (v >= 0) {
          uint4 q = rx[cb][it];
          if (PRO && pact[cb] >= 0) {
            q = XH ? f16x8_to_bf16x8(xform_f16x8(q, psc[cb], psh[cb], pact[cb])) : xform_bf16x8(q, psc[cb], psh[cb], pact[cb]);
            if (!((okm >> it) & 1u)) q = make_uint4(0, 0, 0, 0);
          } else if (XH) {
            q = f16x8_to_bf16x8(q);
          }
          xs[cb * XPS + ((v >> 15) & 0x7fff) * XRS + (v & 0x7fff)] = q;
        }
      }
#pragma unroll
    for (int it = 0; it < D_ITERS; ++it) ds[d_lds0 + (it >> 1) * DPS + 8 * (it & 1) * DRS] = rd[it];
  };

  f32x4 acc[NACC];
#pragma unroll
  for (int a = 0; a < NACC; ++a) acc[a] = (f32x4){0.f, 0.f, 0.f, 0.f};

  const int work = g.N * tiles;
  if (bid < work) prefetch(bid);
  auto tile_loop = [&](auto tg_c) __attribute__((always_inline)) {
  for (int wi = bid; wi < work; wi += gridDim.x) {
    __syncthreads();
    commit();
    __syncthreads();
#ifndef MC_WEXP_NOLOAD
    if (wi + (int)gridDim.x < work) prefetch(wi + gridDim.x);
#endif
#ifdef MC_WEXP_NOK
    if (g.N > 1000000)
#endif
#ifndef MC_WGRAD_ROW_UNROLL
#define MC_WGRAD_ROW_UNROLL 2
#endif
    if constexpr (RS != 0) {
      typedef unsigned int u2 __attribute__((ext_vector_type(2)));
      auto body = [&](auto tg_c) __attribute__((always_inline)) {
        constexpr int TG = decltype(tg_c)::value;
        constexpr int T0 = TG == 0 ? 0 : TPW + (TG - 1) * (TPW - 1);
        constexpr int T1 = (TPW + TG * (TPW - 1)) < KK ? (TPW + TG * (TPW - 1)) : KK;
        static_assert(TG < NS - 1 || (T1 == KK && T1 - T0 < TPW), "the last tap group ends the filter and has a spare slot");
#pragma unroll
        for (int rg = 0; rg < WTH / 4; ++rg) {
#pragma unroll
          for (int cb = 0; cb < NS; ++cb) {
            const short* dp = ds_s + lane_d + (rg * 4 * DRS + cb * 8) * 8;
            bf16x8 a[NTW];
#pragma unroll
            for (int t = 0; t < NTW; ++t) a[t] = tr_frag(dp + t * 2 * DPS * 8);
#pragma unroll
            for (int ky = 0; ky < K; ++ky) {
              if (ky * K + K <= T0 || ky * K >= T1) continue;
              const short* xp = xs_s + lane_x + ((rg * 4 + ky) * XRS + cb * 8) * 8;
              const u2 b0 = __builtin_bit_cast(u2, __builtin_amdgcn_ds_read_tr16_b64_v4i16((lds_v4s*)xp));
              const u2 b1 = __builtin_bit_cast(u2, __builtin_amdgcn_ds_read_tr16_b64_v4i16((lds_v4s*)(xp + 32)));
              const u2 b2 = __builtin_bit_cast(u2, __builtin_amdgcn_ds_read_tr16_b64_v4i16((lds_v4s*)(xp + 64)));
              const unsigned d[6] = {b0[0], b0[1], b1[0], b1[1], b2[0], b2[1]};
#pragma unroll
              for (int kx = 0; kx < K; ++kx) {
                const int tap = ky * K + kx;
                if (tap < T0 || tap >= T1) continue;
                v4u w;
                if (kx % 2 == 0) {
                  w = (v4u){d[kx / 2], d[kx / 2 + 1], d[kx / 2 + 2], d[kx / 2 + 3]};
                } else {
#pragma unroll
                  for (int j = 0; j < 4; ++j) w[j] = __builtin_amdgcn_alignbit(d[kx / 2 + j + 1], d[kx / 2 + j], 16);
                }
#pragma unroll
                for (int t = 0; t < NTW; ++t)
                  acc[(tap - T0) * NTW + t] = __builtin_amdgcn_mfma_f32_16x16x32_bf16(a[t], __builtin_bit_cast(bf16x8, w), acc[(tap - T0) * NTW + t], 0, 0, 0);
              }
            }
            if (TG == NS - 1 && do_bias) {
#pragma unroll
              for (int t = 0; t < NTW; ++t)
                acc[(TPW - 1) * NTW + t] = __builtin_amdgcn_mfma_f32_16x16x32_bf16(a[t], ones, acc[(TPW - 1) * NTW + t], 0, 0, 0);
            }
#ifndef MC_WGRAD_NOFENCE
            if constexpr (NS > 1) __builtin_amdgcn_sched_barrier(0);
#endif
          }
        }
      };
      body(tg_c);
    } else {
#pragma unroll MC_WGRAD_ROW_UNROLL
    for (int row = 0; row < WTH; ++row) {
      bf16x8 a[NTW];
#pragma unroll
      for (int t = 0; t < NTW; ++t) a[t] = tr_frag(ds_s + lane_d + (t * 2 * DPS + row * WTW) * 8);
      if constexpr (NTW >= MC_WGRAD_BATCH_NTW) {
        bf16x8 bq[NTAP];
#pragma unroll
        for (int ti = 0; ti < NTAP; ++ti) bq[ti] = tr_frag(xtap[ti] + row * TIW * 8);
#pragma unroll
        for (int ti = 0; ti < NTAP; ++ti) {
          if (toff[ti] >= 0) {
#pragma unroll
            for (int t = 0; t < NTW; ++t) acc[ti * NTW + t] = __builtin_amdgcn_mfma_f32_16x16x32_bf16(a[t], bq[ti], acc[ti * NTW + t], 0, 0, 0);
          }
        }
      } else {
#pragma unroll
        for (int ti = 0; ti < NTAP; ++ti) {
          if (toff[ti] >= 0) {
            bf16x8 b = tr_frag(xtap[ti] + row * TIW * 8);
#pragma unroll
            for (int t = 0; t < NTW; ++t) acc[ti * NTW + t] = __builtin_amdgcn_mfma_f32_16x16x32_bf16(a[t], b, acc[ti * NTW + t], 0, 0, 0);
          }
        }
      }
      if (do_bias) {
#pragma unroll
        for (int t = 0; t < NTW; ++t)
          acc[(NTAP - 1) * NTW + t] = __builtin_amdgcn_mfma_f32_16x16x32_bf16(a[t], ones, acc[(NTAP - 1) * NTW + t], 0, 0, 0);
      }
    }
    }
  }
  };
  if constexpr (NS == 1) tile_loop(std::integral_constant<int, 0>{});
  else if constexpr (NS == 2) { if (tg == 0) tile_loop(std::integral_constant<int, 0>{}); else tile_loop(std::integral_constant<int, 1>{}); }
  else {
    if (tg == 0) tile_loop(std::integral_constant<int, 0>{}); else if (tg == 1) tile_loop(std::integral_constant<int, 1>{});
    else if (tg == 2) tile_loop(std::integral_constant<int, 2>{}); else tile_loop(std::integral_constant<int, 3>{});
  }
  const int nch = wg_chunks(g.CinP);
  float* pb = part + (size_t)bid * wg_slab_floats(g.CoutP, g.CinP, KK);
  if constexpr (RS != 0) {
    f32x4* red = reinterpret_cast<f32x4*>(smem);
    for (int src = 1; src < NG; ++src) {
      __syncthreads();
      if (cg == src) {
#pragma unroll
        for (int a = 0; a < NACC; ++a) red[(tg * NACC + a) * 64 + lane] = acc[a];
      }
      __syncthreads();
      if (cg == 0) {
#pragma unroll
        for (int a = 0; a < NACC; ++a) acc[a] += red[(tg * NACC + a) * 64 + lane];
      }
    }
    if (cg != 0) return;
    const int t0 = tg == 0 ? 0 : TPW + (tg - 1) * (TPW - 1);
    const int nt = min(KK, TPW + tg * (TPW - 1)) - t0;
#pragma unroll
    for (int sl = 0; sl < TPW; ++sl)
#pragma unroll
      for (int t = 0; t < NTW; ++t)
#pragma unroll
        for (int r = 0; r < 4; ++r) {
          int co = (cog * NTW + t) * 16 + gq * 4 + r;
          if (sl < nt && co < g.CoutP) pb[((size_t)((t0 + sl) * nch + chunk) * g.CoutP + co) * 16 + (lane & 15)] = acc[sl * NTW + t][r];
        }
    if (do_bias && (lane & 15) == 0) {
#pragma unroll
      for (int t = 0; t < NTW; ++t)
#pragma unroll
        for (int r = 0; r < 4; ++r) {
          int co = (cog * NTW + t) * 16 + gq * 4 + r;
          if (co < g.CoutP) pb[(size_t)KK * nch * g.CoutP * 16 + co] = acc[(TPW - 1) * NTW + t][r];
        }
    }
    return;
  }
#pragma unroll
  for (int ti = 0; ti < NTAP; ++ti) {
    int tap = wave + 4 * ti;
#pragma unroll
    for (int t = 0; t < NTW; ++t)
#pragma unroll
      for (int r = 0; r < 4; ++r) {
        int co = (cog * NTW + t) * 16 + gq * 4 + r;
        if (co >= g.CoutP) continue;
        if (tap < KK) {
          pb[((size_t)(tap * nch + chunk) * g.CoutP + co) * 16 + (lane & 15)] = acc[ti * NTW + t][r];
        } else if (do_bias && ti == NTAP - 1 && (lane & 15) == 0) {
          pb[(size_t)KK * nch * g.CoutP * 16 + co] = acc[ti * NTW + t][r];
        }
      }
  }
}

#ifndef MC_NT1_MT
#define MC_NT1_MT 8
#endif
inline Bf16Cfg cfg_for(int c_out, int k, int ho) {
  static const int th12 = getenv("MC_CONV_TH12") ? atoi(getenv("MC_CONV_TH12")) : 1;
  int ntiles = (c_out + 15) / 16;
  int nt = pick_nt(ntiles);
  if (nt == 1) return {16, 32, 1, MC_NT1_MT};
  const bool t12 = th12 && k == 5 && (ho + 11) / 12 * 12 < (ho + 15) / 16 * 16;
  static const int th8 = getenv("MC_CONV_TH8") ? atoi(getenv("MC_CONV_TH8")) : 40;
  if (th8 && k == 5 && ho <= th8) return nt == 2 ? Bf16Cfg{8, 16, 2, 2} : Bf16Cfg{8, 16, 4, 2};
  if (nt == 2) return t12 ? Bf16Cfg{12, 16, 2, 3} : Bf16Cfg{16, 16, 2, 4};
  static const int th24 = getenv("MC_CONV_TH24") ? atoi(getenv("MC_CONV_TH24")) : 80;
  if (th24 && k == 5 && ho <= th24 && (ho + 23) / 24 * 24 <= (t12 ? (ho + 11) / 12 * 12 : (ho + 15) / 16 * 16)) return Bf16Cfg{24, 16, 4, 6};
  return t12 ? Bf16Cfg{12, 16, 4, 3} : Bf16Cfg{16, 16, 4, 4};
}

}

int mc_bf16_tile(const mc_conv_desc* d, int* th, int* tw) {
  Bf16Cfg c = cfg_for(d->c_out, d->k, d->h + 2 * d->pad - d->k + 1);
  *th = c.th; *tw = c.tw;
  return MC_OK;
}

void mc_bf16_bank_dims(const ConvGeom& g, int dgrad, int& chunks, int& steps, int& ntiles) {
  int cb_in = dgrad ? g.CBout : g.CBin;
  int c_out = dgrad ? g.CinP : g.Cout;
  chunks = (cb_in + CHUNK_CB - 1) / CHUNK_CB;
  steps = g.K == 5 ? KSteps<5>::steps : KSteps<3>::steps;
  int nt_total = (c_out + 15) / 16;
  int nt = pick_nt(nt_total);
  ntiles = (nt_total + nt - 1) / nt * nt;
}

size_t mc_bf16_bank_bytes(const ConvGeom& g, int dgrad) {
  int chunks, steps, ntiles;
  mc_bf16_bank_dims(g, dgrad, chunks, steps, ntiles);
  return (size_t)chunks * steps * ntiles * 64 * 16;
}

int mc_bf16_pack(const ConvGeom& g, const float* w, int dgrad, void* packed, hipStream_t s) {
  int chunks, steps, ntiles;
  mc_bf16_bank_dims(g, dgrad, chunks, steps, ntiles);
  size_t total = (size_t)chunks * steps * ntiles * 64 * 8;
  int blocks = (int)((total + 255) / 256);
  if (blocks > 4096) blocks = 4096;
  hipLaunchKernelGGL(k_pack_bf16, dim3(blocks), dim3(256), 0, s, g, w, dgrad, (bf16_t*)packed, chunks, steps, ntiles,
                     (g.dtype == MC_MIX16 && !dgrad) ? 1 : 0);
  MC_CHECK_LAUNCH();
  return MC_OK;
}

const char* mc_bf16_kernel_name(const ConvGeom& g) {
  Bf16Cfg c = cfg_for(g.Cout, g.K, g.Ho);
  if (g.out_f32) return g.K == 5 ? "k_conv_mfma_bf16<5,16,32,1,8,true>" : "k_conv_mfma_bf16<3,16,32,1,8,true>";
  if (g.K == 5 && c.th == 24) return "k_conv_mfma_bf16<5,24,16,4,6,false>";
  if (g.K == 5 && c.th == 12) return c.nt == 2 ? "k_conv_mfma_bf16<5,12,16,2,3,false>" : "k_conv_mfma_bf16<5,12,16,4,6,false,2x2>";
  if (g.K == 5 && c.th == 8) return c.nt == 2 ? "k_conv_mfma_bf16<5,8,16,2,2,false>" : "k_conv_mfma_bf16<5,8,16,4,4,false,2x2>";
  if (g.K == 5) return c.nt == 1 ? "k_conv_mfma_bf16<5,16,32,1,8,false>" : (c.nt == 2 ? "k_conv_mfma_bf16<5,16,16,2,4,false>" : "k_conv_mfma_bf16<5,16,16,4,8,false,2x2>");
  return c.nt == 1 ? "k_conv_mfma_bf16<3,16,32,1,8,false>" : (c.nt == 2 ? "k_conv_mfma_bf16<3,16,16,2,4,false>" : "k_conv_mfma_bf16<3,16,16,4,8,false,2x2>");
}

int mc_conv2d_bf16(const ConvGeom& g_in, const void* x0, const void* x1, const void* bank, const float* bias, void* y0,
                   void* y1, float* part, const ConvFuse& fz, int fuse, hipStream_t s) {
  const ConvGeom& g = g_in;
  Bf16Cfg c = cfg_for(g.Cout, g.K, g.Ho);
  int nt_total = (g.Cout + 15) / 16;
  int groups = (nt_total + c.nt - 1) / c.nt;
  int items = g.tiles * g.N;
  static int cap_total = getenv("MC_CONV_CAP") ? atoi(getenv("MC_CONV_CAP")) : 4096;
  int cap = cap_total / groups > 0 ? cap_total / groups : 1;
  int bx = items < cap ? items : cap;
  dim3 grid(bx, groups, 1);
  if (fuse == 2 && g.out_f32) return MC_EUNSUPPORTED;
  const bool h16 = fuse == 2 ? fz.ey16 != 0 : g.dtype == MC_MIX16;
#define LAUNCH_H(K, TH, TW, NT, MT, F32, FU, H, WN)                                                                    \
  hipLaunchKernelGGL((k_conv_mfma_bf16<K, TH, TW, NT, MT, F32, FU, H, WN>), grid, dim3(64 * (TH * (TW / 16) / (MT)) * (WN)), 0, s, g, \
                     (const bf16_t*)x0, (const bf16_t*)x1, (const bf16_t*)bank, bias, (bf16_t*)y0, (bf16_t*)y1, part,  \
                     groups, fz)
#define LAUNCH_F(K, TH, TW, NT, MT, F32, FU, WN)                                                                       \
  do { if (h16) LAUNCH_H(K, TH, TW, NT, MT, F32, FU, true, WN); else LAUNCH_H(K, TH, TW, NT, MT, F32, FU, false, WN); } while (0)
#define LAUNCH_W(K, TH, TW, NT, MT, F32, WN)                                                                           \
  do { if (fuse == 0) LAUNCH_F(K, TH, TW, NT, MT, F32, 0, WN); else if (fuse == 1) LAUNCH_F(K, TH, TW, NT, MT, F32, 1, WN);   \
       else LAUNCH_F(K, TH, TW, NT, MT, false, 2, WN); } while (0)
#define LAUNCH(K, TH, TW, NT, MT, F32) LAUNCH_W(K, TH, TW, NT, MT, F32, 1)
  static const int wn2 = getenv("MC_CONV_WN") ? atoi(getenv("MC_CONV_WN")) : 2;
#define LAUNCH4(K, TH, TW, MT) do { if (wn2 == 2) LAUNCH_W(K, TH, TW, 4, 2 * (MT), false, 2); else LAUNCH_W(K, TH, TW, 4, MT, false, 1); } while (0)
  if (g.out_f32) {
    if (g.K == 5) LAUNCH(5, 16, 32, 1, MC_NT1_MT, true); else if (g.K == 3) LAUNCH(3, 16, 32, 1, MC_NT1_MT, true); else return MC_EUNSUPPORTED;
  } else if (g.K == 5) {
    if (c.nt == 1) LAUNCH(5, 16, 32, 1, MC_NT1_MT, false);
    else if (c.th == 24) LAUNCH_W(5, 24, 16, 4, 6, false, 1);
    else if (c.th == 12) { if (c.nt == 2) LAUNCH(5, 12, 16, 2, 3, false); else LAUNCH4(5, 12, 16, 3); }
    else if (c.th == 8) { if (c.nt == 2) LAUNCH(5, 8, 16, 2, 2, false); else LAUNCH4(5, 8, 16, 2); }
    else if (c.nt == 2) LAUNCH(5, 16, 16, 2, 4, false); else LAUNCH4(5, 16, 16, 4);
  } else if (g.K == 3) {
    if (c.nt == 1) LAUNCH(3, 16, 32, 1, MC_NT1_MT, false); else if (c.nt == 2) LAUNCH(3, 16, 16, 2, 4, false); else LAUNCH4(3, 16, 16, 4);
  } else {
    return MC_EUNSUPPORTED;
  }
#undef LAUNCH4
#undef LAUNCH_W
#undef LAUNCH
#undef LAUNCH_F
#undef LAUNCH_H
  MC_CHECK_LAUNCH();
  return MC_OK;
}

int mc_wgrad_bf16(const ConvGeom& g_in, const void* x0, const void* x1, const void* dy, void* part, const ConvFuse& fz,
                  int fuse, hipStream_t s) {
  const ConvGeom& g = g_in;
  const int tiles_x = (g.Wo + WTW - 1) / WTW, tiles_y = (g.Ho + WTH - 1) / WTH;
  const int tiles = tiles_x * tiles_y;
  const int ntiles = (g.Cout + 15) / 16;
  const int ntw = pick_nt(ntiles) >= 2 ? 2 : 1;
  dim3 grid(g.wgrad_G, (g.CBin + 1) / 2, (ntiles + ntw - 1) / ntw);
  const bool xh = g.dtype == MC_MIX16;
#define WLAUNCH_X(K, NTW, RS, PRO, XH)                                                                                 \
  hipLaunchKernelGGL((k_wgrad_mfma_bf16<K, NTW, RS, PRO, XH>), grid, dim3(256), 0, s, g, (const bf16_t*)x0, (const bf16_t*)x1, \
                     (const bf16_t*)dy, (float*)part, tiles_x, tiles, fz)
#define WLAUNCH_P(K, NTW, RS, PRO) do { if (xh) WLAUNCH_X(K, NTW, RS, PRO, true); else WLAUNCH_X(K, NTW, RS, PRO, false); } while (0)
#define WLAUNCH(K, NTW, RS) do { if (fuse) WLAUNCH_P(K, NTW, RS, true); else WLAUNCH_P(K, NTW, RS, false); } while (0)
  static const int rs = [] { const char* e = getenv("MC_WGRAD_RS"); return e ? atoi(e) : 44; }();
  const int v = ntw == 1 ? rs / 10 : rs % 10;
#define WPICK(K, NTW) do { if (v == 4) WLAUNCH(K, NTW, 4); else if (v == 2) WLAUNCH(K, NTW, 2); else if (v == 1 && NTW == 1) WLAUNCH(K, 1, 1); else WLAUNCH(K, NTW, 0); } while (0)
  if (g.K == 5) { if (ntw == 1) WPICK(5, 1); else WPICK(5, 2); }
  else if (g.K == 3) { if (ntw == 1) WPICK(3, 1); else WPICK(3, 2); }
  else return MC_EUNSUPPORTED;
#undef WPICK
#undef WLAUNCH
#undef WLAUNCH_P
#undef WLAUNCH_X
  MC_CHECK_LAUNCH();
  return MC_OK;
}
```

### pbml_mantle_convection_amd/csrc/conv_common.h

```cpp
#pragma once
#include <stdlib.h>
#include "common.h"

struct ConvGeom {
  int N, H, W, Ho, Wo, K, pad, pad_mode;
  int Cin0, Cin1, Cin;
  int CB0, CB1, CBin, CinP;
  int Cout, CBout, CoutP;
  int split8;
  int tiles_x, tiles_y, tiles;
  int wgrad_G;
  int sym_h, U;
  int nh, nv, nq;
  int dtype;
  int out_f32;
};

struct ConvFuse {
  const float* coef0; const float* coef1;
  int act0, act1;
  const void* ey;
  const float* ecoef;
  float* epart;
  int eact, epad, ezero, ehs, ews;
  int estride;
  int ey16;
};
static inline ConvFuse conv_fuse_none() {
  ConvFuse f;
  f.coef0 = f.coef1 = nullptr; f.act0 = f.act1 = MC_ACT_NONE;
  f.ey = nullptr; f.ecoef = nullptr; f.epart = nullptr; f.eact = MC_ACT_NONE; f.epad = 0; f.ezero = 1; f.ehs = f.ews = 0; f.estride = 0;
  f.ey16 = 0;
  return f;
}

static __host__ __device__ inline int wg_chunks(int CinP) { return (CinP + 15) / 16; }
static __host__ __device__ inline size_t wg_slab_floats(int CoutP, int CinP, int KK) {
  return (size_t)KK * wg_chunks(CinP) * CoutP * 16 + CoutP;
}
static __host__ __device__ inline size_t wg_index(int tap, int cip, int co, int CoutP, int nch) {
  return ((size_t)(tap * nch + (cip >> 4)) * CoutP + co) * 16 + (cip & 15);
}
static inline long wgrad_target_blocks2() {
  static long v = 0;
  if (!v) { const char* e = getenv("MC_WGRAD_BLOCKS2"); v = e ? atol(e) : 512; if (v < 16) v = 16; }
  return v;
}
static inline long wgrad_min_slabs() {
  static long v = 0;
  if (!v) { const char* e = getenv("MC_WGRAD_MIN_G"); v = e ? atol(e) : 16; if (v < 1) v = 1; }
  return v;
}
static inline long wgrad_target_blocks() {
  static long v = 0;
  if (!v) { const char* e = getenv("MC_WGRAD_BLOCKS"); v = e ? atol(e) : 768; if (v < 16) v = 16; }
  return v;
}

static inline int conv_geom(const mc_conv_desc* d, int tile_h, int tile_w, ConvGeom& g) {
  if (!d) return MC_EINVAL;
  if (d->n <= 0 || d->h <= 0 || d->w <= 0 || d->c_in0 <= 0 || d->c_in1 < 0 || d->c_out <= 0) return MC_EINVAL;
  if (d->k != 3 && d->k != 5) return MC_EUNSUPPORTED;
  if (d->pad < 0 || d->pad > d->k - 1) return MC_EINVAL;
  if (d->pad_mode < MC_PAD_ZEROS || d->pad_mode > MC_PAD_REFLECT) return MC_EINVAL;
  if (d->pad_mode == MC_PAD_REFLECT && (d->pad >= d->h || d->pad >= d->w)) return MC_EINVAL;
  if (d->c_in1 > 0 && (d->c_in0 % 8) != 0) return MC_EUNSUPPORTED;
  if (d->sym_h < 0 || (d->sym_h & 1) || d->sym_v < 0 || (d->sym_v & 1) || d->sym_hv < 0 || (d->sym_hv & 3) ||
      d->sym_h + d->sym_v + d->sym_hv > d->c_out)
    return MC_EINVAL;
  if (d->c_out_split != 0 && (d->c_out_split < 0 || d->c_out_split >= d->c_out || (d->c_out_split % 8) != 0))
    return MC_EINVAL;
  g.N = d->n; g.H = d->h; g.W = d->w; g.K = d->k; g.pad = d->pad; g.pad_mode = d->pad_mode;
  g.Ho = d->h + 2 * d->pad - d->k + 1;
  g.Wo = d->w + 2 * d->pad - d->k + 1;
  if (g.Ho <= 0 || g.Wo <= 0) return MC_EINVAL;
  g.Cin0 = d->c_in0; g.Cin1 = d->c_in1; g.Cin = d->c_in0 + d->c_in1;
  g.CB0 = (d->c_in0 + 7) / 8; g.CB1 = (d->c_in1 + 7) / 8; g.CBin = g.CB0 + g.CB1; g.CinP = g.CBin * 8;
  g.Cout = d->c_out; g.CBout = (d->c_out + 7) / 8; g.CoutP = g.CBout * 8;
  g.split8 = d->c_out_split / 8;
  g.tiles_x = (g.Wo + tile_w - 1) / tile_w;
  g.tiles_y = (g.Ho + tile_h - 1) / tile_h;
  g.tiles = g.tiles_x * g.tiles_y;
  g.sym_h = d->sym_h; g.nh = d->sym_h / 2; g.nv = d->sym_v / 2; g.nq = d->sym_hv / 4;
  g.U = d->c_out - g.nh - g.nv - 3 * g.nq;
  g.dtype = d->dtype;
  g.out_f32 = mc_is16(d->dtype) ? d->out_f32 : 0;
  if (g.out_f32 < 0 || g.out_f32 > 1) return MC_EINVAL;
  if (g.out_f32 && (d->c_out > 16 || d->c_out_split != 0)) return MC_EUNSUPPORTED;
  long slab = (long)wg_slab_floats(g.CoutP, g.CinP, g.K * g.K) * 4;
  long cap = (64L << 20) / slab;
  if (cap < 32) cap = 32;
  long G, work;
  if (mc_is16(g.dtype)) {
    int ntiles = (g.Cout + 15) / 16;
    int ntw = (ntiles % 2 == 0) ? 2 : 1;
    long other = (long)((g.CBin + 1) / 2) * ((ntiles + ntw - 1) / ntw);
    const long target = ntw == 1 ? wgrad_target_blocks() : wgrad_target_blocks2();
    G = ntw == 1 ? (target + other - 1) / other : target / other;
    if (G < wgrad_min_slabs()) G = wgrad_min_slabs();
    work = (long)g.N * ((g.Ho + 15) / 16) * ((g.Wo + 31) / 32);
  } else {
    G = 1024;
    work = (long)g.N * g.tiles;
  }
  if (G > cap) G = cap;
  if (G > work) G = work;
  g.wgrad_G = (int)G;
  return MC_OK;
}

static __host__ __device__ inline int cin_padded_index(int ci, int Cin0, int CB0) {
  return ci < Cin0 ? ci : CB0 * 8 + (ci - Cin0);
}

template <typename G>
__host__ __device__ __forceinline__ int mirror_source(const G& g, int co, bool& fx, bool& fy) {
  fx = fy = false;
  if (co < g.U) return co;
  int j = co - g.U;
  if (j < g.nh) { fx = true; return j; }
  j -= g.nh;
  if (j < g.nv) { fy = true; return g.nh + j; }
  j -= g.nv;
  const int blk = g.nq > 0 ? j / g.nq : 0;
  fx = blk == 0 || blk == 2; fy = blk == 1 || blk == 2;
  return g.nh + g.nv + (g.nq > 0 ? j % g.nq : 0);
}
template <typename G>
__device__ __forceinline__ float bank_source(const G& g, const float* __restrict__ wu, int co, int cip, int ky, int kx) {
  int ob = cip / 8, oj = cip % 8;
  bool ok = co < g.Cout && ob < g.CBin && (ob < g.CB0 ? (ob * 8 + oj < g.Cin0) : ((ob - g.CB0) * 8 + oj < g.Cin1));
  if (!ok) return 0.f;
  int ci = ob < g.CB0 ? ob * 8 + oj : g.Cin0 + (ob - g.CB0) * 8 + oj;
  const int cw = g.Cin;
  bool fx, fy;
  const int u = mirror_source(g, co, fx, fy);
  const int kxs = fx ? g.K - 1 - kx : kx, kys = fy ? g.K - 1 - ky : ky;
  return wu[(((size_t)u * cw + ci) * g.K + kys) * g.K + kxs];
}

template <typename G>
__device__ __forceinline__ float pack_value_f32(const G& g, const float* __restrict__ wu, size_t i, int dgrad) {
  const int K = g.K, KK = K * K;
  const int cop = dgrad ? g.CinP : g.CoutP;
  int o = (int)(i % cop);
  size_t r = i / cop;
  int j = (int)(r % 8); r /= 8;
  int tap = (int)(r % KK);
  int cb = (int)(r / KK);
  if (!dgrad) return bank_source(g, wu, o, cb * 8 + j, tap / K, tap % K);
  return bank_source(g, wu, cb * 8 + j, o, K - 1 - tap / K, K - 1 - tap % K);
}

template <typename G>
__device__ __forceinline__ float pack_value_bf16(const G& g, const float* __restrict__ wu, size_t i, int dgrad, int steps,
                                                 int ntiles) {
  const int K = g.K, KK = K * K;
  int e = (int)(i & 7);
  int lane = (int)((i >> 3) & 63);
  size_t r = i >> 9;
  int nt = (int)(r % ntiles); r /= ntiles;
  int s = (int)(r % steps);
  int ck = (int)(r / steps);
  int n = lane & 15, gq = lane >> 4;
  int j = 4 * s + gq;
  int tap = j / 2, cb = j % 2;
  if (tap >= KK) return 0.f;
  int kin = ck * 16 + cb * 8 + e, kout = nt * 16 + n;
  int ky = tap / K, kx = tap % K;
  if (!dgrad) return bank_source(g, wu, kout, kin, ky, kx);
  return bank_source(g, wu, kin, kout, K - 1 - ky, K - 1 - kx);
}
```

### pbml_mantle_convection_amd/csrc/conv_rr_bf16.hip

```cpp
#include "conv_rr.h"
#include <type_traits>

using bf16x8 = __attribute__((ext_vector_type(8))) short;
using f16x8 = __attribute__((ext_vector_type(8))) _Float16;
using f32x4 = __attribute__((ext_vector_type(4))) float;
typedef unsigned int v4u __attribute__((ext_vector_type(4)));

#ifdef MC_RR_STAMPS
#define RR_STAMP(k) do { __builtin_amdgcn_sched_barrier(0); long long now_ = clock64(); st_acc[k] += now_ - st_prev; st_prev = now_; __builtin_amdgcn_sched_barrier(0); } while (0)
#else
#define RR_STAMP(k) do {} while (0)
#endif

namespace {

__device__ __forceinline__ int rr_xcd_remap(int bid, int nwg) {
  const int xcd = bid & 7, q = nwg >> 3, r = nwg & 7;
  return (xcd < r ? xcd * (q + 1) : r * (q + 1) + (xcd - r) * q) + (bid >> 3);
}

__global__ void k_pack_rr(ConvGeom g, const float* __restrict__ wu, int dgrad, bf16_t* __restrict__ bank, int ntiles, size_t total, int f16) {
  for (size_t i = blockIdx.x * (size_t)blockDim.x + threadIdx.x; i < total; i += (size_t)gridDim.x * blockDim.x) {
    const float v = rr_pack_value(g, wu, i, dgrad, ntiles);
    bank[i] = f16 ? __builtin_bit_cast(bf16_t, (_Float16)v) : f2bf(v);
  }
}

template <bool H16> __device__ __forceinline__ f32x4 rr_mfma(bf16x8 a, bf16x8 b, f32x4 c) {
  if constexpr (H16) return __builtin_amdgcn_mfma_f32_16x16x32_f16(__builtin_bit_cast(f16x8, a), __builtin_bit_cast(f16x8, b), c, 0, 0, 0);
  else return __builtin_amdgcn_mfma_f32_16x16x32_bf16(a, b, c, 0, 0, 0);
}
template <bool H16> __device__ __forceinline__ uint32_t rr_pk(float a, float b) {
  if constexpr (H16) return pk_f16(a, b);
  else return pk_bf16(a, b);
}

template <int K, int FUSE, bool OUT_F32, bool GELU, bool H16 = false, bool DZM = false>
__global__ __launch_bounds__(512, 2) void k_conv_rr_bf16(ConvGeom g, const bf16_t* __restrict__ x0, const bf16_t* __restrict__ x1,
                                                         const bf16_t* __restrict__ bank, const float* __restrict__ bias,
                                                         bf16_t* __restrict__ y0, bf16_t* __restrict__ y1,
                                                         float* __restrict__ part, ConvFuse fz) {
  using S = RR<K>;
  static_assert(!DZM || (FUSE == 2 && H16 && GELU), "the MFMA-side dz epilogue is the packed-f16 GELU form");
  constexpr bool LEX = FUSE == 2 && !DZM;
  constexpr int TIH = S::TIH, TIW = S::TIW, PLANE = S::PLANE, NFRAG = S::NFRAG, NTY = S::NTYPES;
  constexpr int PER = (TIH * TIW + 255) / 256;
  constexpr int YSLOTS = RR_R * RR_TW, YPER = YSLOTS / 256;
  constexpr int NW = LEX ? 1 : 2;
  extern __shared__ __attribute__((aligned(16))) char smem_raw[];
  uint4* const inbuf = reinterpret_cast<uint4*>(smem_raw);
  uint4* const wbuf = inbuf + 2 * 2 * PLANE;
  uint4* const exch = wbuf;

  const int grp = blockIdx.y;
  const int ntiles_total = gridDim.y;
  const int bid = rr_xcd_remap(blockIdx.x, gridDim.x);
  const int lane = threadIdx.x & 63, wave = __builtin_amdgcn_readfirstlane(threadIdx.x >> 6);
  const int chunks = (g.CBin + 1) / 2;
  const int items = g.N * g.tiles;
  const int my_items = (items - bid + (int)gridDim.x - 1) / (int)gridDim.x;
  const int total = my_items * chunks;
  if (total <= 0) return;
  const bool w_global = LEX && chunks > 1;

  auto stage_coords = [&](int t, int& n, int& ty0, int& tx0, int& ck, int& tile) {
    const int jitem = t / chunks;
    ck = t - jitem * chunks;
    const int wi = bid + jitem * (int)gridDim.x;
    n = wi / g.tiles;
    tile = wi - n * g.tiles;
    ty0 = (tile / g.tiles_x) * RR_R;
    tx0 = (tile % g.tiles_x) * RR_TW;
  };
  if (wave >= RR_STRIPS) {
    const int tl = threadIdx.x - 64 * RR_STRIPS;
    int s_rc[PER];
    unsigned s_off[PER];
#pragma unroll
    for (int it = 0; it < PER; ++it) {
      int i = tl + it * 256;
      const bool live = i < TIH * TIW;
      if (!live) i = TIH * TIW - 1;
      const int r = i / TIW, c = i - r * TIW;
      s_rc[it] = (live ? 0 : (1 << 31)) | (r << 15) | c;
      s_off[it] = (unsigned)(r * g.W + c) * 16u;
    }
    constexpr int NSET = LEX ? 1 : 2;
    v4u rin[NSET][2][PER];
    unsigned okm[2] = {0xffffffffu, 0xffffffffu};
    v4u yv[2][YPER];
    float ecv[4] = {1.f, 0.f, 0.f, 0.f};
    constexpr int WPER = (NFRAG * 64 + 255) / 256;
    v4u wv[LEX ? 1 : 2][LEX ? 1 : WPER];
    const bool w_every = !w_global && chunks > 1;

    auto issue = [&](int t, auto set_c) {
      constexpr int SET = decltype(set_c)::value;
      int n, ty0, tx0, ck, tile;
      stage_coords(t, n, ty0, tx0, ck, tile);
      const bool interior = (ty0 - g.pad >= 0) && (ty0 - g.pad + TIH <= g.H) && (tx0 - g.pad >= 0) && (tx0 - g.pad + TIW <= g.W);
      const unsigned org16 = (unsigned)((ty0 - g.pad) * g.W + (tx0 - g.pad)) * 16u;
      okm[SET] = 0xffffffffu;
#pragma unroll
      for (int cb = 0; cb < 2; ++cb) {
        const int gcb = ck * 2 + cb;
        const int gcc = min(gcb, g.CBin - 1);
        const bool second = gcc >= g.CB0;
        int scb = second ? gcc - g.CB0 : gcc;
        int sC8 = second ? g.CB1 : g.CB0;
        const void* sp = second ? (const void*)x1 : (const void*)x0;
        const size_t plane_bytes = (size_t)g.H * g.W * 16;
        const char* pbase = reinterpret_cast<const char*>(sp) + ((size_t)n * sC8 + scb) * plane_bytes;
        __amdgpu_buffer_rsrc_t rs = __builtin_amdgcn_make_buffer_rsrc((void*)pbase, 0, gcb < g.CBin ? (int)plane_bytes : 0, 0x00020000);
#pragma unroll
        for (int it = 0; it < PER; ++it) {
          unsigned off;
          if (interior) {
            off = org16 + s_off[it];
          } else {
            const int r = (s_rc[it] >> 15) & 0x7fff, c = s_rc[it] & 0x7fff;
            bool oky, okx;
            const int sy = pad_map_sel(ty0 + r - g.pad, g.H, g.pad_mode, oky);
            const int sx = pad_map_sel(tx0 + c - g.pad, g.W, g.pad_mode, okx);
            off = (oky && okx) ? (unsigned)(sy * g.W + sx) * 16u : 0xFFFFFFF0u;
            if (FUSE == 1 && cb == 0 && !(oky && okx)) okm[SET] &= ~(1u << it);
          }
          rin[SET][cb][it] = __builtin_amdgcn_raw_buffer_load_b128(rs, off, 0, 0);
        }
      }
      if constexpr (!LEX) {
        if (!w_global && (w_every || t == 0)) {
          const v4u* wsrc = reinterpret_cast<const v4u*>(bank) + (size_t)(ck * ntiles_total + grp) * NFRAG * 64;
#pragma unroll
          for (int it = 0; it < WPER; ++it) wv[SET][it] = wsrc[min(tl + it * 256, NFRAG * 64 - 1)];
        }
      }
    };
    auto load_y = [&](int t) {
      if constexpr (LEX) {
        if ((t % chunks) != chunks - 1) return;
        int n, ty0, tx0, ck, tile;
        stage_coords(t, n, ty0, tx0, ck, tile);
        const bf16_t* ey = reinterpret_cast<const bf16_t*>(fz.ey);
#pragma unroll
        for (int cb = 0; cb < 2; ++cb) {
          const int cbc = min(grp * 2 + cb, g.CBout - 1);
#pragma unroll
          for (int it = 0; it < YPER; ++it) {
            const int i = tl + it * 256, r = i / RR_TW, c = i - r * RR_TW;
            const int cy = min(max(ty0 + r - fz.epad, 0), fz.ehs - 1), cx = min(max(tx0 + c - fz.epad, 0), fz.ews - 1);
            yv[cb][it] = *reinterpret_cast<const v4u*>(ey + cb8_index(n, cbc, cy, cx, g.CBout, fz.ehs, fz.ews));
          }
        }
        ecv[0] = 1.f; ecv[1] = 0.f; ecv[2] = 0.f; ecv[3] = 0.f;
        if (fz.ecoef) {
          const float4 c4 = reinterpret_cast<const float4*>(fz.ecoef)[(size_t)n * g.CoutP + min(grp * 16 + (lane & 15), g.CoutP - 1)];
          ecv[0] = c4.x; ecv[1] = c4.y; ecv[2] = c4.z; ecv[3] = c4.w;
        }
      }
    };
    auto epilogue_dz = [&](int t) {
      if constexpr (LEX) {
        if ((t % chunks) != chunks - 1) return;
        int n, ty0, tx0, ck, tile;
        stage_coords(t, n, ty0, tx0, ck, tile);
        const int p = fz.epad, fr = fz.ezero ? 0 : p + 1;
        float s[2][16];
#pragma unroll
        for (int cb = 0; cb < 2; ++cb)
#pragma unroll
          for (int j = 0; j < 16; ++j) s[cb][j] = 0.f;
        bf16_t* yout = y0;
        bool inb[YPER], fin[YPER];
        int pix[YPER];
        size_t oidx[YPER];
#pragma unroll
        for (int it = 0; it < YPER; ++it) {
          const int i = tl + it * 256, r = i / RR_TW, c = i - r * RR_TW;
          const int oy = ty0 + r, ox = tx0 + c, iy = oy - p, ix = ox - p;
          pix[it] = i;
          inb[it] = oy < g.Ho && ox < g.Wo;
          fin[it] = inb[it] && iy >= fr && iy < fz.ehs - fr && ix >= fr && ix < fz.ews - fr;
          oidx[it] = cb8_index(n, grp * 2, min(oy, g.Ho - 1), min(ox, g.Wo - 1), g.CBout, g.Ho, g.Wo);
        }
#pragma unroll
        for (int cb = 0; cb < 2; ++cb) {
          float da[YPER][8], o[YPER][8];
#pragma unroll
          for (int it = 0; it < YPER; ++it) {
            const int sw = (pix[it] >> 2) & 3;
            const f32x4 a0 = reinterpret_cast<const f32x4*>(exch)[pix[it] * 4 + ((2 * cb) ^ sw)];
            const f32x4 a1 = reinterpret_cast<const f32x4*>(exch)[pix[it] * 4 + ((2 * cb + 1) ^ sw)];
            da[it][0] = a0[0]; da[it][1] = a0[1]; da[it][2] = a0[2]; da[it][3] = a0[3];
            da[it][4] = a1[0]; da[it][5] = a1[1]; da[it][6] = a1[2]; da[it][7] = a1[3];
          }
#pragma unroll
          for (int h = 0; h < 4; ++h) {
            float c0[4], c1[4];
#pragma unroll
            for (int q = 0; q < 4; ++q) {
              c0[q] = __builtin_bit_cast(float, __builtin_amdgcn_readlane(__builtin_bit_cast(int, ecv[q]), 8 * cb + 2 * h));
              c1[q] = __builtin_bit_cast(float, __builtin_amdgcn_readlane(__builtin_bit_cast(int, ecv[q]), 8 * cb + 2 * h + 1));
              asm volatile("" : "+v"(c0[q]), "+v"(c1[q]));
            }
#pragma unroll
            for (int it = 0; it < YPER; ++it) {
              const unsigned yw = yv[cb][it][h];
              const f32x2 yy = H16 ? unpk_f16(yw) : (f32x2){__uint_as_float(yw << 16), __uint_as_float(yw & 0xffff0000u)};
              const f32x2 z = pk_fma(yy, (f32x2){c0[0], c1[0]}, (f32x2){c0[1], c1[1]});
              f32x2 gp;
              if (GELU || fz.eact == MC_ACT_GELU) gp = gelu_grad_poly2(z);
              else gp = (f32x2){act_bwd(z.x, fz.eact), act_bwd(z.y, fz.eact)};
              const f32x2 dA = (f32x2){da[it][2 * h], da[it][2 * h + 1]};
              const f32x2 dz = dA * gp;
              const f32x2 yh = (yy - (f32x2){c0[2], c1[2]}) * (f32x2){c0[3], c1[3]};
              if (fin[it]) {
                s[cb][4 * h] += dz.x; s[cb][4 * h + 1] += dz.x * yh.x;
                s[cb][4 * h + 2] += dz.y; s[cb][4 * h + 3] += dz.y * yh.y;
              }
              o[it][2 * h] = fin[it] ? dz.x : dA.x; o[it][2 * h + 1] = fin[it] ? dz.y : dA.y;
            }
          }
          if (grp * 2 + cb < g.CBout) {
#pragma unroll
            for (int it = 0; it < YPER; ++it)
              if (inb[it])
                *reinterpret_cast<uint4*>(yout + oidx[it] + (size_t)cb * g.Ho * g.Wo * 8) =
                    make_uint4(pk_bf16(o[it][0], o[it][1]), pk_bf16(o[it][2], o[it][3]), pk_bf16(o[it][4], o[it][5]), pk_bf16(o[it][6], o[it][7]));
          }
        }
#pragma unroll
        for (int cb = 0; cb < 2; ++cb) {
          int idx;
          const float tot = wave_sum16(s[cb], lane, idx);
          const int co = grp * 16 + cb * 8 + (idx >> 1);
          if ((lane & 3) == 0 && co < g.CoutP)
            fz.epart[(((size_t)n * fz.estride + (size_t)tile * RR_STRIPS + (wave - RR_STRIPS)) * g.CoutP + co) * 2 + (idx & 1)] = tot;
        }
      }
    };
    auto commit = [&](int t, auto set_c) {
      constexpr int SET = decltype(set_c)::value;
      int n, ty0, tx0, ck, tile;
      stage_coords(t, n, ty0, tx0, ck, tile);
      uint4* dst = inbuf + (t & 1) * 2 * PLANE;
#pragma unroll
      for (int cb = 0; cb < 2; ++cb) {
        uint4 v[PER];
#pragma unroll
        for (int it = 0; it < PER; ++it) v[it] = make_uint4(rin[SET][cb][it][0], rin[SET][cb][it][1], rin[SET][cb][it][2], rin[SET][cb][it][3]);
        if constexpr (FUSE == 1) {
          const int gcb = ck * 2 + cb;
          const bool second = gcb >= g.CB0;
          const float* ct = second ? fz.coef1 : fz.coef0;
          const int pact = second ? fz.act1 : fz.act0;
          if (gcb < g.CBin && (ct != nullptr || pact != MC_ACT_NONE)) {
            float psc[8], psh[8];
            load_coef8(ct, n, (second ? g.CB1 : g.CB0) * 8, second ? gcb - g.CB0 : gcb, psc, psh);
#pragma unroll
            for (int it = 0; it < PER; ++it)
              v[it] = H16 ? xform_f16x8(v[it], psc, psh, GELU ? (int)MC_ACT_GELU : pact) : xform_bf16x8(v[it], psc, psh, GELU ? (int)MC_ACT_GELU : pact);
            if (okm[SET] != 0xffffffffu) {
#pragma unroll
              for (int it = 0; it < PER; ++it) if (!((okm[SET] >> it) & 1u)) v[it] = make_uint4(0, 0, 0, 0);
            }
          }
        }
#pragma unroll
        for (int it = 0; it < PER; ++it)
          if (s_rc[it] >= 0) dst[cb * PLANE + ((s_rc[it] >> 15) & 0x7fff) * TIW + (s_rc[it] & 0x7fff)] = v[it];
      }
      if constexpr (!LEX) {
        if (!w_global && (w_every || t == 0)) {
          v4u* wd = reinterpret_cast<v4u*>(wbuf) + (w_every ? (t & 1) : 0) * NFRAG * 64;
#pragma unroll
          for (int it = 0; it < WPER; ++it) if (tl + it * 256 < NFRAG * 64) wd[tl + it * 256] = wv[SET][it];
        }
      }
    };
    using S0 = std::integral_constant<int, 0>;
    using S1 = std::integral_constant<int, 1>;
#ifdef MC_RR_STAMPS
    long long st_acc[4] = {0, 0, 0, 0}, st_prev = clock64();
#endif
    if constexpr (LEX) {
      if (!w_global) {
        const v4u* wsrc = reinterpret_cast<const v4u*>(bank) + (size_t)grp * NFRAG * 64;
        v4u* wd = reinterpret_cast<v4u*>(wbuf);
#pragma unroll
        for (int it = 0; it < WPER; ++it) {
          const v4u w = wsrc[min(tl + it * 256, NFRAG * 64 - 1)];
          if (tl + it * 256 < NFRAG * 64) wd[tl + it * 256] = w;
        }
      }
      issue(0, S0{});
      commit(0, S0{});
      __syncthreads();
      for (int t = 0; t <= total; ++t) {
        if (t + 1 < total) issue(t + 1, S0{});
        RR_STAMP(3);
        if (t > 0) epilogue_dz(t - 1);
        if (t == total) break;
        load_y(t);
        RR_STAMP(0);
        if (t + 1 < total) commit(t + 1, S0{});
        RR_STAMP(1);
        __syncthreads();
        __syncthreads();
        RR_STAMP(2);
      }
#ifdef MC_RR_STAMPS
      if (blockIdx.x == 77 && blockIdx.y == 0 && threadIdx.x == 256)
        printf("loader (dz) stages %d: epilogue + y loads %lld commit %lld barriers %lld issue %lld\n", total, st_acc[0], st_acc[1], st_acc[2], st_acc[3]);
#endif
      return;
    } else {
    issue(0, S0{});
    if (total > 1) issue(1, std::integral_constant<int, NSET - 1>{});
    commit(0, S0{});
    __syncthreads();
    RR_STAMP(3);
    for (int t = 0; t < total; t += 2) {
      if (t + 2 < total) issue(t + 2, S0{});
      RR_STAMP(0);
      if (t + 1 < total) commit(t + 1, S1{});
      RR_STAMP(1);
      __syncthreads();
      RR_STAMP(2);
      if (t + 1 >= total) break;
      if (t + 3 < total) issue(t + 3, S1{});
      RR_STAMP(0);
      if (t + 2 < total) commit(t + 2, S0{});
      RR_STAMP(1);
      __syncthreads();
      RR_STAMP(2);
    }
    }
#ifdef MC_RR_STAMPS
    if (blockIdx.x == 77 && blockIdx.y == 0 && threadIdx.x == 256)
      printf("loader stages %d: issue %lld commit %lld barrier %lld prologue %lld\n", total, st_acc[0], st_acc[1], st_acc[2], st_acc[3]);
#endif
    return;
  }

  const int strip = wave;
  const int m = lane & 15, gq = lane >> 4;
  int aoff[NTY];
#pragma unroll
  for (int T = 0; T < NTY; ++T) {
    int rho = S::rho(T, 0), kx = S::kx(T, 0), cb = S::cb(T, 0);
#pragma unroll
    for (int gg = 1; gg < 4; ++gg) if (gq == gg) { rho = S::rho(T, gg); kx = S::kx(T, gg); cb = S::cb(T, gg); }
    aoff[T] = cb * PLANE + rho * TIW + kx + strip * 16 + m;
  }
  float bv[4];
#pragma unroll
  for (int r = 0; r < 4; ++r) {
    const int co = grp * 16 + gq * 4 + r;
    bv[r] = (bias && co < g.Cout) ? bias[co] : 0.f;
  }
  f32x4 acc[RR_R];
  bf16x8 wf[NFRAG];
  const int cob = grp * 2 + (gq >> 1);
  const bool cobok = cob < g.CBout;
  const int cbc = min(cob, g.CBout - 1);
  const int tiles4 = g.tiles * RR_STRIPS;

  __syncthreads();
#ifdef MC_RR_STAMPS
  long long st_acc[6] = {0, 0, 0, 0, 0, 0}, st_prev = clock64();
#endif

  for (int t = 0; t < total; ++t) {
    int n, ty0, tx0, ck, tile;
    stage_coords(t, n, ty0, tx0, ck, tile);
    if (ck == 0) {
#pragma unroll
      for (int r = 0; r < RR_R; ++r) acc[r] = (f32x4){bv[0], bv[1], bv[2], bv[3]};
    }
    if (!DZM && chunks == 1 && t > 0) {
    } else if (w_global) {
      const uint4* wsrc = reinterpret_cast<const uint4*>(bank) + ((size_t)(ck * ntiles_total + grp) * NFRAG) * 64 + lane;
#pragma unroll
      for (int f = 0; f < NFRAG; ++f) wf[f] = __builtin_bit_cast(bf16x8, wsrc[(size_t)f * 64]);
    } else {
      const uint4* ws = wbuf + ((NW == 2 && chunks > 1) ? (t & 1) : 0) * NFRAG * 64 + lane;
#pragma unroll
      for (int f = 0; f < NFRAG; ++f) wf[f] = __builtin_bit_cast(bf16x8, ws[f * 64]);
    }
    v4u yl[DZM ? RR_R / 2 : 1];
    if constexpr (DZM) {
      const bf16_t* ey = reinterpret_cast<const bf16_t*>(fz.ey);
      const int cx = min(max(tx0 + strip * 16 + m - fz.epad, 0), fz.ews - 1);
#pragma unroll
      for (int r = 0; r < RR_R; r += 2) {
        const int cy = min(max(ty0 + r + (gq & 1) - fz.epad, 0), fz.ehs - 1);
        yl[r / 2] = *reinterpret_cast<const v4u*>(ey + cb8_index(n, cbc, cy, cx, g.CBout, fz.ehs, fz.ews));
      }
    }
    RR_STAMP(0);
    const uint4* buf = inbuf + (t & 1) * 2 * PLANE;
    constexpr int NF = (TIH / 2) * NTY, AHEAD = 3;
    bf16x8 fr[4];
    auto ldf = [&](int k) { return *reinterpret_cast<const bf16x8*>(buf + aoff[k % NTY] + 2 * (k / NTY) * TIW); };
#pragma unroll
    for (int k = 0; k < AHEAD; ++k) fr[k] = ldf(k);
#pragma unroll
    for (int k = 0; k < NF; ++k) {
      if (k + AHEAD < NF) fr[(k + AHEAD) & 3] = ldf(k + AHEAD);
      const int T = k % NTY, i = 2 * (k / NTY);
#pragma unroll
      for (int kappa = S::kmin(T); kappa <= S::kmax(T); ++kappa) {
        const int r = i - kappa;
        if (r >= 0 && r < RR_R) acc[r] = rr_mfma<(H16 && FUSE != 2)>(wf[S::fidx(T, kappa)], fr[k & 3], acc[r]);
      }
      __builtin_amdgcn_sched_barrier(0);
    }
    RR_STAMP(1);
    if constexpr (LEX) {
      __syncthreads();
      if (ck == chunks - 1) {
#pragma unroll
        for (int r = 0; r < RR_R; ++r) {
          const int pix = r * RR_TW + strip * 16 + m;
          reinterpret_cast<f32x4*>(exch)[pix * 4 + (gq ^ ((pix >> 2) & 3))] = acc[r];
        }
      }
    }
    RR_STAMP(4);
    if (!LEX && ck == chunks - 1) {
      const int ox = tx0 + strip * 16 + m;
      f32x2 s1[2] = {(f32x2){0.f, 0.f}, (f32x2){0.f, 0.f}}, s2[2] = {(f32x2){0.f, 0.f}, (f32x2){0.f, 0.f}};
      if constexpr (DZM) {
        typedef _Float16 h2 __attribute__((ext_vector_type(2)));
        const int p = fz.epad, fr_ = fz.ezero ? 0 : p + 1;
        const int ix = ox - p;
        const bool colok = ox < g.Wo && cobok;
        const bool colfin = colok && ix >= fr_ && ix < fz.ews - fr_;
        float csc[4] = {1.f, 1.f, 1.f, 1.f}, csh[4] = {0.f, 0.f, 0.f, 0.f}, cme[4] = {0.f, 0.f, 0.f, 0.f}, crs[4] = {0.f, 0.f, 0.f, 0.f};
        if (fz.ecoef) {
#pragma unroll
          for (int r = 0; r < 4; ++r) {
            const float4 c4 = reinterpret_cast<const float4*>(fz.ecoef)[(size_t)n * g.CoutP + cbc * 8 + (gq & 1) * 4 + r];
            csc[r] = c4.x; csh[r] = c4.y; cme[r] = c4.z; crs[r] = c4.w;
          }
        }
        const h2 sc01 = __builtin_bit_cast(h2, pk_f16(csc[0], csc[1])), sc23 = __builtin_bit_cast(h2, pk_f16(csc[2], csc[3]));
        const h2 sh01 = __builtin_bit_cast(h2, pk_f16(csh[0], csh[1])), sh23 = __builtin_bit_cast(h2, pk_f16(csh[2], csh[3]));
        float zero = 0.f;
        asm volatile("" : "+v"(zero));
        float sd[4] = {0.f, 0.f, 0.f, 0.f}, sy[4] = {0.f, 0.f, 0.f, 0.f};
        char* dst16 = reinterpret_cast<char*>(y0) + (cb8_index(n, cbc, ty0, ox, g.CBout, g.Ho, g.Wo)) * 2 + (size_t)(gq & 1) * g.Wo * 16;
        const size_t row_bytes = (size_t)g.Wo * 16;
        const int iy0 = ty0 - p;
        auto rows = [&](auto full_c) {
          constexpr bool FULL = decltype(full_c)::value;
#pragma unroll
          for (int r = 0; r < RR_R; r += 2) {
            const unsigned l0 = yl[r / 2][0], l1 = yl[r / 2][1], l2 = yl[r / 2][2], l3 = yl[r / 2][3];
            const auto u01 = __builtin_amdgcn_permlane16_swap(l0, l2, false, false);
            const auto u23 = __builtin_amdgcn_permlane16_swap(l1, l3, false, false);
            h2 yy[4] = {__builtin_bit_cast(h2, (unsigned)u01[0]), __builtin_bit_cast(h2, (unsigned)u23[0]),
                        __builtin_bit_cast(h2, (unsigned)u01[1]), __builtin_bit_cast(h2, (unsigned)u23[1])};
            h2 zc[4], w[4], q[4], gg[4];
            const h2 R = {(_Float16)3.0f, (_Float16)3.0f};
#pragma unroll
            for (int c = 0; c < 4; ++c) zc[c] = __builtin_elementwise_fma(yy[c], (c & 1) ? sc23 : sc01, (c & 1) ? sh23 : sh01);
#pragma unroll
            for (int c = 0; c < 4; ++c) zc[c] = __builtin_elementwise_max(zc[c], -R);
#pragma unroll
            for (int c = 0; c < 4; ++c) zc[c] = __builtin_elementwise_min(zc[c], R);
#pragma unroll
            for (int c = 0; c < 4; ++c) w[c] = zc[c] * zc[c];
#pragma unroll
            for (int c = 0; c < 4; ++c)
              q[c] = __builtin_elementwise_fma((h2){(_Float16)1.3422040e-04f, (_Float16)1.3422040e-04f}, w[c],
                                               (h2){(_Float16)-3.8080227e-03f, (_Float16)-3.8080227e-03f});
#pragma unroll
            for (int c = 0; c < 4; ++c) q[c] = __builtin_elementwise_fma(q[c], w[c], (h2){(_Float16)4.2797559e-02f, (_Float16)4.2797559e-02f});
#pragma unroll
            for (int c = 0; c < 4; ++c) q[c] = __builtin_elementwise_fma(q[c], w[c], (h2){(_Float16)-2.4320666e-01f, (_Float16)-2.4320666e-01f});
#pragma unroll
            for (int c = 0; c < 4; ++c) q[c] = __builtin_elementwise_fma(q[c], w[c], (h2){(_Float16)7.8907706e-01f, (_Float16)7.8907706e-01f});
#pragma unroll
            for (int c = 0; c < 4; ++c) gg[c] = __builtin_elementwise_fma(zc[c], q[c], (h2){(_Float16)0.5f, (_Float16)0.5f});
            h2 gm[4], ge[4], hy[4];
#pragma unroll
            for (int c = 0; c < 4; ++c) {
              gm[c] = gg[c]; ge[c] = gg[c];
              if constexpr (!FULL) {
                const int iy = iy0 + r + (c >> 1);
                const bool fin = colfin && ty0 + r + (c >> 1) < g.Ho && iy >= fr_ && iy < fz.ehs - fr_;
                gm[c] = fin ? gg[c] : (h2){(_Float16)0.f, (_Float16)0.f};
                ge[c] = fin ? gg[c] : (h2){(_Float16)1.f, (_Float16)1.f};
              }
            }
#pragma unroll
            for (int c = 0; c < 4; ++c) hy[c] = gm[c] * yy[c];
            unsigned pk[4];
#pragma unroll
            for (int c = 0; c < 4; ++c) {
              const float dA0 = acc[r + (c >> 1)][2 * (c & 1)], dA1 = acc[r + (c >> 1)][2 * (c & 1) + 1];
              const float dz0 = __builtin_fmaf(dA0, (float)ge[c].x, zero), dz1 = __builtin_fmaf(dA1, (float)ge[c].y, zero);
              sd[2 * (c & 1)] = __builtin_fmaf(dA0, (float)gm[c].x, sd[2 * (c & 1)]);
              sd[2 * (c & 1) + 1] = __builtin_fmaf(dA1, (float)gm[c].y, sd[2 * (c & 1) + 1]);
              sy[2 * (c & 1)] = __builtin_fmaf(dA0, (float)hy[c].x, sy[2 * (c & 1)]);
              sy[2 * (c & 1) + 1] = __builtin_fmaf(dA1, (float)hy[c].y, sy[2 * (c & 1) + 1]);
              pk[c] = pk_bf16(dz0, dz1);
            }
            const auto sx = __builtin_amdgcn_permlane16_swap(pk[0], pk[2], false, false);
            const auto sz = __builtin_amdgcn_permlane16_swap(pk[1], pk[3], false, false);
            if (FULL || (colok && ty0 + r + (gq & 1) < g.Ho))
              *reinterpret_cast<uint4*>(dst16 + (size_t)r * row_bytes) = make_uint4(sx[0], sz[0], sx[1], sz[1]);
          }
        };
        if (ty0 + RR_R <= g.Ho && tx0 + RR_TW <= g.Wo && grp * 2 + 1 < g.CBout && iy0 >= fr_ && iy0 + RR_R <= fz.ehs - fr_ &&
            tx0 - p >= fr_ && tx0 - p + RR_TW <= fz.ews - fr_)
          rows(std::true_type{});
        else
          rows(std::false_type{});
#pragma unroll
        for (int c = 0; c < 4; ++c) sy[c] = crs[c] * (sy[c] - cme[c] * sd[c]);
        s1[0] = (f32x2){sd[0], sd[1]}; s1[1] = (f32x2){sd[2], sd[3]};
        s2[0] = (f32x2){sy[0], sy[1]}; s2[1] = (f32x2){sy[2], sy[3]};
      } else {
      constexpr int esz = OUT_F32 ? 4 : 2;
      char* dst;
      if (g.split8 > 0 && cbc >= g.split8)
        dst = reinterpret_cast<char*>(y1) + (cb8_index(n, cbc - g.split8, ty0, ox, g.CBout - g.split8, g.Ho, g.Wo) + (gq & 1) * 4) * esz;
      else
        dst = reinterpret_cast<char*>(y0) + (cb8_index(n, cbc, ty0, ox, g.split8 > 0 ? g.split8 : g.CBout, g.Ho, g.Wo) + (gq & 1) * 4) * esz;
      const size_t row_bytes = (size_t)g.Wo * 8 * esz;
      const bool colok = ox < g.Wo && cobok;
      if constexpr (OUT_F32) {
        {
#pragma unroll
        for (int r = 0; r < RR_R; ++r) {
          const f32x2 v01 = (f32x2){acc[r][0], acc[r][1]}, v23 = (f32x2){acc[r][2], acc[r][3]};
          if (colok && ty0 + r < g.Ho) {
            s1[0] += v01; s1[1] += v23;
            s2[0] = pk_fma(v01, v01, s2[0]); s2[1] = pk_fma(v23, v23, s2[1]);
            *reinterpret_cast<float4*>(dst + (size_t)r * row_bytes) = make_float4(v01.x, v01.y, v23.x, v23.y);
          }
        }
        }
      } else {
        char* dst16 = dst - (gq & 1) * 4 * esz + (size_t)(gq & 1) * row_bytes;
        auto rows = [&](auto full_c) {
          constexpr bool FULL = decltype(full_c)::value;
#pragma unroll
          for (int r = 0; r < RR_R; r += 2) {
            const f32x2 a01 = (f32x2){acc[r][0], acc[r][1]}, a23 = (f32x2){acc[r][2], acc[r][3]};
            const f32x2 b01 = (f32x2){acc[r + 1][0], acc[r + 1][1]}, b23 = (f32x2){acc[r + 1][2], acc[r + 1][3]};
            if (FULL || (colok && ty0 + r < g.Ho)) {
              s1[0] += a01; s1[1] += a23;
              s2[0] = pk_fma(a01, a01, s2[0]); s2[1] = pk_fma(a23, a23, s2[1]);
            }
            if (FULL || (colok && ty0 + r + 1 < g.Ho)) {
              s1[0] += b01; s1[1] += b23;
              s2[0] = pk_fma(b01, b01, s2[0]); s2[1] = pk_fma(b23, b23, s2[1]);
            }
            const auto sx = __builtin_amdgcn_permlane16_swap(rr_pk<H16>(a01.x, a01.y), rr_pk<H16>(b01.x, b01.y), false, false);
            const auto sy = __builtin_amdgcn_permlane16_swap(rr_pk<H16>(a23.x, a23.y), rr_pk<H16>(b23.x, b23.y), false, false);
#ifdef MC_RR_NOSTORE
            if ((FULL || (colok && ty0 + r + (gq & 1) < g.Ho)) && sx[0] == 0x12345678u)
#else
            if (FULL || (colok && ty0 + r + (gq & 1) < g.Ho))
#endif
              *reinterpret_cast<uint4*>(dst16 + (size_t)r * row_bytes) = make_uint4(sx[0], sy[0], sx[1], sy[1]);
          }
        };
        if (ty0 + RR_R <= g.Ho && tx0 + RR_TW <= g.Wo && grp * 2 + 1 < g.CBout) rows(std::true_type{});
        else rows(std::false_type{});
      }
      }
      RR_STAMP(5);
      float* pp = DZM ? fz.epart : part;
      const int slots = DZM ? fz.estride : tiles4;
      if (pp) {
        float q8[8] = {s1[0].x, s2[0].x, s1[0].y, s2[0].y, s1[1].x, s2[1].x, s1[1].y, s2[1].y};
#pragma unroll
        for (int k = 0; k < 8; ++k) {
          q8[k] += __builtin_bit_cast(float, __builtin_amdgcn_update_dpp(0, __builtin_bit_cast(int, q8[k]), 0x128, 0xf, 0xf, false));
          q8[k] += __builtin_bit_cast(float, __builtin_amdgcn_update_dpp(0, __builtin_bit_cast(int, q8[k]), 0x124, 0xf, 0xf, false));
          q8[k] += __builtin_bit_cast(float, __builtin_amdgcn_update_dpp(0, __builtin_bit_cast(int, q8[k]), 0x122, 0xf, 0xf, false));
          q8[k] += __builtin_bit_cast(float, __builtin_amdgcn_update_dpp(0, __builtin_bit_cast(int, q8[k]), 0x121, 0xf, 0xf, false));
        }
        float q1 = q8[0];
#pragma unroll
        for (int k = 1; k < 8; ++k) q1 = (m >> 1) == k ? q8[k] : q1;
        const int co = grp * 16 + gq * 4 + (m >> 2);
        if ((m & 1) == 0 && co < g.CoutP) {
          pp[(((size_t)n * slots + (size_t)tile * RR_STRIPS + strip) * g.CoutP + co) * 2 + ((m >> 1) & 1)] = q1;
        }
      }
    }
    RR_STAMP(2);
    __syncthreads();
    RR_STAMP(3);
  }
#ifdef MC_RR_STAMPS
  if (blockIdx.x == 77 && blockIdx.y == 0 && threadIdx.x == 0)
    printf("mfma stages %d: wload %lld kloop %lld exch %lld rows %lld stats %lld barrier %lld\n", total, st_acc[0], st_acc[1], st_acc[4], st_acc[5], st_acc[2], st_acc[3]);
#endif
}

}

bool mc_rr_applies(int dtype, int cout, int wo, bool full_pad) {
  const int ntiles = (cout + 15) / 16;
  static const int on = [] { const char* e = getenv("MC_CONV_RR"); return e ? atoi(e) : 2; }();
  static const int minw = [] { const char* e = getenv("MC_RR_MINW"); return e ? atoi(e) : 100; }();
  static const int minw_full = [] { const char* e = getenv("MC_RR_MINW_DGRAD"); return e ? atoi(e) : 140; }();
  if (!on || !mc_is16(dtype)) return false;
  if (full_pad && minw_full > 0 && wo < minw_full) return false;
  if (ntiles % 2 == 1) return true;
  return on >= 2 && ntiles <= 8 && wo >= minw;
}

void mc_rr_tile(int* th, int* tw) { *th = RR_R; *tw = RR_TW; }
int mc_rr_stat_slots(const ConvGeom& g) { return g.tiles * RR_STRIPS; }

static void rr_bank_dims(const ConvGeom& g, int dgrad, int& chunks, int& ntiles, int& nfrag) {
  const int cb_in = dgrad ? g.CBout : g.CBin;
  const int c_out = dgrad ? g.CinP : g.Cout;
  chunks = (cb_in + 1) / 2;
  ntiles = (c_out + 15) / 16;
  nfrag = g.K == 5 ? RR<5>::NFRAG : RR<3>::NFRAG;
}
size_t mc_rr_bank_bytes(const ConvGeom& g, int dgrad) {
  int chunks, ntiles, nfrag;
  rr_bank_dims(g, dgrad, chunks, ntiles, nfrag);
  return (size_t)chunks * ntiles * nfrag * 64 * 16;
}
int mc_rr_pack(const ConvGeom& g, const float* w, int dgrad, void* packed, hipStream_t s) {
  int chunks, ntiles, nfrag;
  rr_bank_dims(g, dgrad, chunks, ntiles, nfrag);
  const size_t total = (size_t)chunks * ntiles * nfrag * 64 * 8;
  int blocks = (int)((total + 255) / 256);
  if (blocks > 4096) blocks = 4096;
  hipLaunchKernelGGL(k_pack_rr, dim3(blocks), dim3(256), 0, s, g, w, dgrad, (bf16_t*)packed, ntiles, total,
                     (g.dtype == MC_MIX16 && !dgrad) ? 1 : 0);
  MC_CHECK_LAUNCH();
  return MC_OK;
}

const char* mc_rr_kernel_name(const ConvGeom& g, int fuse) {
  if (g.K == 5) return g.out_f32 ? "k_conv_rr_bf16<5,f32out>" : (fuse == 2 ? "k_conv_rr_bf16<5,dz>" : (fuse == 1 ? "k_conv_rr_bf16<5,norm>" : "k_conv_rr_bf16<5>"));
  return g.out_f32 ? "k_conv_rr_bf16<3,f32out>" : (fuse == 2 ? "k_conv_rr_bf16<3,dz>" : (fuse == 1 ? "k_conv_rr_bf16<3,norm>" : "k_conv_rr_bf16<3>"));
}

template <int K, int FUSE, bool F32, bool GELU, bool H16 = false, bool DZM = false>
static int rr_launch(const ConvGeom& g, const void* x0, const void* x1, const void* bank, const float* bias, void* y0, void* y1,
                     float* part, const ConvFuse& fz, hipStream_t s) {
  using S = RR<K>;
  constexpr bool LEX = FUSE == 2 && !DZM;
  const size_t lds = (size_t)2 * 2 * S::PLANE * 16 + (LEX ? (size_t)RR_R * RR_TW * 64 : (size_t)2 * S::NFRAG * 1024);
  static bool attr_dev[64] = {};
  int dev = 0;
  if (hipGetDevice(&dev) != hipSuccess || dev < 0 || dev >= 64) return MC_EINVAL;
  bool& attr_set = attr_dev[dev];
  if (!attr_set) {
    hipError_t e = hipFuncSetAttribute(reinterpret_cast<const void*>(&k_conv_rr_bf16<K, FUSE, F32, GELU, H16, DZM>),
                                       hipFuncAttributeMaxDynamicSharedMemorySize, (int)lds);
    if (e != hipSuccess) return (int)e;
    attr_set = true;
  }
  const int groups = (g.Cout + 15) / 16;
  const int items = g.tiles * g.N;
  static const int cap_total = [] { const char* e = getenv("MC_RR_CAP"); return e ? atoi(e) : 256; }();
  int cap = cap_total / groups > 0 ? cap_total / groups : 1;
  const int bx = items < cap ? items : cap;
  hipLaunchKernelGGL((k_conv_rr_bf16<K, FUSE, F32, GELU, H16, DZM>), dim3(bx, groups, 1), dim3(512), lds, s, g, (const bf16_t*)x0,
                     (const bf16_t*)x1, (const bf16_t*)bank, bias, (bf16_t*)y0, (bf16_t*)y1, part, fz);
  MC_CHECK_LAUNCH();
  return MC_OK;
}

int mc_conv2d_rr(const ConvGeom& g, const void* x0, const void* x1, const void* bank, const float* bias, void* y0, void* y1,
                 float* part, const ConvFuse& fz, int fuse, hipStream_t s) {
  if (g.K != 5 && g.K != 3) return MC_EUNSUPPORTED;
  if (fuse == 2 && g.out_f32) return MC_EUNSUPPORTED;
  const bool gelu = fuse == 2 ? fz.eact == MC_ACT_GELU
                              : ((fz.act0 == MC_ACT_GELU || (fz.act0 == MC_ACT_NONE && !fz.coef0)) &&
                                 (fz.act1 == MC_ACT_GELU || (fz.act1 == MC_ACT_NONE && !fz.coef1)));
  const bool h16 = fuse == 2 ? fz.ey16 != 0 : g.dtype == MC_MIX16;
#define RRL(K, FU, F32, GE, H) rr_launch<K, FU, F32, GE, H>(g, x0, x1, bank, bias, y0, y1, part, fz, s)
#define RRK(K, H)                                                                                               \
  do {                                                                                                          \
    if (fuse == 0) return g.out_f32 ? RRL(K, 0, true, true, H) : RRL(K, 0, false, true, H);                     \
    if (fuse == 2) return gelu ? RRL(K, 2, false, true, H) : RRL(K, 2, false, false, H);                        \
    if (g.out_f32) return gelu ? RRL(K, 1, true, true, H) : RRL(K, 1, true, false, H);                          \
    return gelu ? RRL(K, 1, false, true, H) : RRL(K, 1, false, false, H);                                       \
  } while (0)
  if (h16 && fuse == 2 && gelu && g.CBin <= 2) {
    if (g.K == 5) return rr_launch<5, 2, false, true, true, true>(g, x0, x1, bank, bias, y0, y1, part, fz, s);
    return rr_launch<3, 2, false, true, true, true>(g, x0, x1, bank, bias, y0, y1, part, fz, s);
  }
  if (h16) { if (g.K == 5) RRK(5, true); RRK(3, true); }
  if (g.K == 5) RRK(5, false);
  RRK(3, false);
#undef RRK
#undef RRL
}
```

Baseline: 3194 samples/s.

## Split dgrad-style RR convs into aligned main region plus small-tile tail launch

For 16-bit convolutions with full padding (pad = k-1) on the RR path, the output is split into a main region aligned to the RR tile sizes and thin leftover strips along the right and bottom edges. The main region runs the RR kernel and the strips run the generic bf16 kernel with a new smaller 16x16 tail tile config. Packed weight banks now hold a second bf16 bank for the tail, and the GN stat slots are remapped so the tail zeroes its own partial slots. The aim is to avoid running whole RR tiles over mostly out-of-bounds edge work, at the cost of an extra kernel launch per conv and a larger weight bank.

```diff
diff --git a/include/mantle_hip.h b/include/mantle_hip.h
--- a/include/mantle_hip.h
+++ b/include/mantle_hip.h
@@ -72,6 +72,16 @@
   int32_t y_f16;
 } mc_conv_epilogue;
 
+typedef struct {
+  int32_t split;
+  int32_t main_h, main_w;
+  int32_t main_tiles_y, main_tiles_x;
+  int32_t slots, main_slots;
+  int32_t tail_tile_h, tail_tile_w;
+  int32_t tail_rect[2][4];
+  int32_t tail_tiles_col, tail_tiles_row;
+} mc_conv_plan;
+
 int mc_version(void);
 const char* mc_strerror(int code);
 
@@ -88,6 +98,7 @@
                     void* stream);
 const char* mc_conv_kernel_name(const mc_conv_desc* d);
 int32_t mc_conv_tiles(const mc_conv_desc* d);
+int mc_conv_launch_plan(const mc_conv_desc* desc, const mc_conv_epilogue* epi, mc_conv_plan* plan);
 int mc_conv2d(const mc_conv_desc* d, const void* x0, const void* x1, const void* packed_w,
               const float* bias, void* y0, void* y1, float* stat_partials, void* stream);
 int mc_conv2d_fused(const mc_conv_desc* d, const void* x0, const void* x1, const mc_conv_prologue* pro,
diff --git a/pbml_mantle_convection_amd/_lib.py b/pbml_mantle_convection_amd/_lib.py
--- a/pbml_mantle_convection_amd/_lib.py
+++ b/pbml_mantle_convection_amd/_lib.py
@@ -35,6 +35,13 @@
                 ("y_f16", C.c_int32)]
 
 
+class ConvPlan(C.Structure):
+    _fields_ = [("split", C.c_int32), ("main_h", C.c_int32), ("main_w", C.c_int32), ("main_tiles_y", C.c_int32),
+                ("main_tiles_x", C.c_int32), ("slots", C.c_int32), ("main_slots", C.c_int32), ("tail_tile_h", C.c_int32),
+                ("tail_tile_w", C.c_int32), ("tail_rect", (C.c_int32 * 4) * 2), ("tail_tiles_col", C.c_int32),
+                ("tail_tiles_row", C.c_int32)]
+
+
 class LossDesc(C.Structure):
     _fields_ = [("n", C.c_int32), ("h", C.c_int32), ("w", C.c_int32), ("p_pred", C.c_int32),
                 ("loss_type", C.c_int32), ("loss_scale", C.c_int32), ("loss_derivative", C.c_int32),
@@ -58,6 +65,7 @@
     "mc_pack_weights": (C.c_int, [_CD, _vp, _i32, _vp, _vp]),
     "mc_conv_tiles": (_i32, [_CD]),
     "mc_conv_kernel_name": (C.c_char_p, [_CD]),
+    "mc_conv_launch_plan": (C.c_int, [_CD, _CE, C.POINTER(ConvPlan)]),
     "mc_conv2d": (C.c_int, [_CD, _vp, _vp, _vp, _vp, _vp, _vp, _vp, _vp]),
     "mc_conv2d_fused": (C.c_int, [_CD, _vp, _vp, _CP, _vp, _vp, _vp, _vp, _vp, _CE, _vp]),
     "mc_conv2d_wgrad_fused": (C.c_int, [_CD, _vp, _vp, _CP, _vp, _vp, _vp]),
diff --git a/pbml_mantle_convection_amd/csrc/conv_api.hip b/pbml_mantle_convection_amd/csrc/conv_api.hip
--- a/pbml_mantle_convection_amd/csrc/conv_api.hip
+++ b/pbml_mantle_convection_amd/csrc/conv_api.hip
@@ -4,7 +4,7 @@
                   void* y1, float* part, const ConvFuse& fz, int fuse, hipStream_t s);
 int mc_wgrad_f32(const ConvGeom& g, const void* x0, const void* x1, const void* dy, void* part, const ConvFuse& fz, int fuse,
                  hipStream_t s);
-int mc_bf16_tile(const mc_conv_desc* d, int* th, int* tw);
+int mc_bf16_tile(const mc_conv_desc* d, bool tail, int* th, int* tw);
 size_t mc_bf16_bank_bytes(const ConvGeom& g, int dgrad);
 int mc_bf16_pack(const ConvGeom& g, const float* w_unique, int dgrad, void* packed, hipStream_t s);
 int mc_conv2d_bf16(const ConvGeom& g, const void* x0, const void* x1, const void* bank, const float* bias, void* y0,
@@ -32,15 +32,63 @@
   if (mc_is16(d->dtype)) {
     if (rr_desc(d)) { th = RR_R; tw = RR_TW; }
     else {
-      int rc = mc_bf16_tile(d, &th, &tw);
+      int rc = mc_bf16_tile(d, false, &th, &tw);
       if (rc) return rc;
     }
   } else if (d->dtype != MC_F32) {
     return MC_EUNSUPPORTED;
   }
-  return conv_geom(d, th, tw, g);
-}
-int stat_slots(const mc_conv_desc* d, const ConvGeom& g) { return rr_desc(d) ? g.tiles * RR_STRIPS : g.tiles; }
+  int rc = conv_geom(d, th, tw, g);
+  if (!rc && mc_is16(d->dtype) && rr_desc(d)) g.slots = g.tiles * RR_STRIPS;
+  return rc;
+}
+int stat_slots(const mc_conv_desc*, const ConvGeom& g) { return g.slots; }
+
+bool dgrad_tail_on() {
+  static const int v = [] { const char* e = getenv("MC_DGRAD_TAIL"); return e ? atoi(e) : 1; }();
+  return v != 0;
+}
+int dgrad_tail_maxw() {
+  static const int v = [] { const char* e = getenv("MC_DGRAD_TAIL_W"); return e ? atoi(e) : 16; }();
+  return v;
+}
+int dgrad_tail_maxh() {
+  static const int v = [] { const char* e = getenv("MC_DGRAD_TAIL_H"); return e ? atoi(e) : 4; }();
+  return v;
+}
+bool bank_has_tail(const ConvGeom& g, int dgrad) { return dgrad_tail_on() && (dgrad || g.pad == g.K - 1); }
+
+int plan_for(const mc_conv_desc* d, const ConvGeom& g, const mc_conv_epilogue* epi, mc_conv_plan& pl) {
+  pl = mc_conv_plan{};
+  pl.main_h = g.Ho; pl.main_w = g.Wo; pl.main_tiles_y = g.tiles_y; pl.main_tiles_x = g.tiles_x;
+  pl.slots = pl.main_slots = g.slots;
+  if (!dgrad_tail_on() || !mc_is16(d->dtype) || d->pad != d->k - 1 || !rr_desc(d) || d->out_f32) return MC_OK;
+  const int remw = g.Wo % RR_TW, remh = g.Ho % RR_R;
+  bool cols = remw > 0 && remw <= dgrad_tail_maxw() && g.Wo > RR_TW;
+  bool rows = remh > 0 && remh <= dgrad_tail_maxh() && g.Ho > RR_R;
+  if (epi) {
+    if (epi->pad_mode == MC_PAD_ZEROS || epi->pad == 0) return MC_OK;
+    cols = cols && g.Wo - remw >= epi->ws - 1;
+    rows = rows && g.Ho - remh >= epi->hs - 1;
+  }
+  if (!cols && !rows) return MC_OK;
+  int th, tw;
+  mc_bf16_tile(d, true, &th, &tw);
+  pl.split = 1;
+  if (cols) { pl.main_w = g.Wo - remw; pl.main_tiles_x = pl.main_w / RR_TW; }
+  if (rows) { pl.main_h = g.Ho - remh; pl.main_tiles_y = pl.main_h / RR_R; }
+  pl.main_slots = pl.main_tiles_x * pl.main_tiles_y * RR_STRIPS;
+  pl.tail_tile_h = th; pl.tail_tile_w = tw;
+  if (cols) {
+    pl.tail_rect[0][0] = 0; pl.tail_rect[0][1] = pl.main_w; pl.tail_rect[0][2] = g.Ho; pl.tail_rect[0][3] = remw;
+    pl.tail_tiles_col = ((g.Ho + th - 1) / th) * ((remw + tw - 1) / tw);
+  }
+  if (rows) {
+    pl.tail_rect[1][0] = pl.main_h; pl.tail_rect[1][1] = 0; pl.tail_rect[1][2] = remh; pl.tail_rect[1][3] = pl.main_w;
+    pl.tail_tiles_row = ((remh + th - 1) / th) * ((pl.main_w + tw - 1) / tw);
+  }
+  return MC_OK;
+}
 
 __global__ void k_pack_f32(ConvGeom g, const float* __restrict__ wu, int dgrad, float* __restrict__ bank, size_t total) {
   for (size_t i = blockIdx.x * (size_t)blockDim.x + threadIdx.x; i < total; i += (size_t)gridDim.x * blockDim.x)
@@ -197,7 +245,7 @@
 size_t mc_packed_weight_bytes(const mc_conv_desc* d, int32_t dgrad) {
   ConvGeom g;
   if (geom_for(d, g)) return 0;
-  if (bank_is_rr(g, dgrad)) return mc_rr_bank_bytes(g, dgrad);
+  if (bank_is_rr(g, dgrad)) return mc_rr_bank_bytes(g, dgrad) + (bank_has_tail(g, dgrad) ? mc_bf16_bank_bytes(g, dgrad) : 0);
   if (mc_is16(g.dtype)) return mc_bf16_bank_bytes(g, dgrad);
   int cbin = dgrad ? g.CBout : g.CBin, cop = dgrad ? g.CinP : g.CoutP;
   return (size_t)cbin * g.K * g.K * 8 * cop * sizeof(float);
@@ -208,7 +256,11 @@
   int rc = geom_for(d, g);
   if (rc) return rc;
   if (!w_unique || !packed) return MC_EINVAL;
-  if (bank_is_rr(g, dgrad)) return mc_rr_pack(g, w_unique, dgrad, packed, (hipStream_t)stream);
+  if (bank_is_rr(g, dgrad)) {
+    rc = mc_rr_pack(g, w_unique, dgrad, packed, (hipStream_t)stream);
+    if (rc || !bank_has_tail(g, dgrad)) return rc;
+    return mc_bf16_pack(g, w_unique, dgrad, (char*)packed + mc_rr_bank_bytes(g, dgrad), (hipStream_t)stream);
+  }
   if (mc_is16(g.dtype)) return mc_bf16_pack(g, w_unique, dgrad, packed, (hipStream_t)stream);
   size_t total = mc_packed_weight_bytes(d, dgrad) / sizeof(float);
   int blocks = (int)((total + 255) / 256);
@@ -266,9 +318,49 @@
     fz.estride = epi->part_stride;
     fuse = 2;
   }
+  mc_conv_plan pl;
+  plan_for(d, g, epi, pl);
+  if (pl.split && !stat_partials) {
+    ConvGeom gm = g;
+    gm.oye = pl.main_h; gm.oxe = pl.main_w;
+    gm.tiles_x = pl.main_tiles_x; gm.tiles_y = pl.main_tiles_y;
+    gm.tiles = gm.tiles_a = gm.tiles_x * gm.tiles_y;
+    rc = mc_conv2d_rr(gm, x0, x1, packed_w, bias, y0, y1, nullptr, fz, fuse, (hipStream_t)stream);
+    if (rc) return rc;
+    ConvGeom gt;
+    rc = conv_geom(d, pl.tail_tile_h, pl.tail_tile_w, gt);
+    if (rc) return rc;
+    gt.tail = 1;
+    const int32_t* ra = pl.tail_rect[pl.tail_tiles_col ? 0 : 1];
+    gt.oy0 = ra[0]; gt.ox0 = ra[1]; gt.oye = ra[0] + ra[2]; gt.oxe = ra[1] + ra[3];
+    gt.tiles_x = (ra[3] + pl.tail_tile_w - 1) / pl.tail_tile_w;
+    gt.tiles_a = pl.tail_tiles_col ? pl.tail_tiles_col : pl.tail_tiles_row;
+    gt.tiles = pl.tail_tiles_col + pl.tail_tiles_row;
+    if (gt.tiles > gt.tiles_a) {
+      const int32_t* rb = pl.tail_rect[1];
+      gt.by0 = rb[0]; gt.bx0 = rb[1]; gt.bye = rb[0] + rb[2]; gt.bxe = rb[1] + rb[3];
+      gt.tiles_xb = (rb[3] + pl.tail_tile_w - 1) / pl.tail_tile_w;
+    }
+    ConvFuse ft = fz;
+    if (fuse == 2) {
+      ft = conv_fuse_none();
+      ft.epart = fz.epart; ft.estride = fz.estride;
+      gt.zslot0 = pl.main_slots; gt.zslots = pl.slots - pl.main_slots;
+    }
+    return mc_conv2d_bf16(gt, x0, x1, (const char*)packed_w + mc_rr_bank_bytes(g, 0), bias, y0, y1, nullptr, ft,
+                          fuse == 2 ? 0 : fuse, (hipStream_t)stream);
+  }
   if (rr_desc(d)) return mc_conv2d_rr(g, x0, x1, packed_w, bias, y0, y1, stat_partials, fz, fuse, (hipStream_t)stream);
   if (mc_is16(g.dtype)) return mc_conv2d_bf16(g, x0, x1, packed_w, bias, y0, y1, stat_partials, fz, fuse, (hipStream_t)stream);
   return mc_conv2d_f32(g, x0, x1, packed_w, bias, y0, y1, stat_partials, fz, fuse, (hipStream_t)stream);
+}
+
+int mc_conv_launch_plan(const mc_conv_desc* d, const mc_conv_epilogue* epi, mc_conv_plan* plan) {
+  ConvGeom g;
+  int rc = geom_for(d, g);
+  if (rc) return rc;
+  if (!plan) return MC_EINVAL;
+  return plan_for(d, g, epi, *plan);
 }
 
 int mc_conv2d(const mc_conv_desc* d, const void* x0, const void* x1, const void* packed_w, const float* bias, void* y0,
@@ -283,7 +375,14 @@
   if (rr_desc(d)) {
     const size_t nfrag = g.K == 5 ? RR<5>::NFRAG : RR<3>::NFRAG;
     const size_t chunks = (g.CBin + 1) / 2, groups = (g.Cout + 15) / 16;
-    return (((chunks - 1) * groups + (groups - 1)) * nfrag * 64 + (nfrag * 64 - 1)) * 16 + 16;
+    const size_t rr_ext = (((chunks - 1) * groups + (groups - 1)) * nfrag * 64 + (nfrag * 64 - 1)) * 16 + 16;
+    mc_conv_plan pl;
+    plan_for(d, g, nullptr, pl);
+    if (!pl.split) return rr_ext;
+    int wchunks, steps, ntiles;
+    mc_bf16_bank_dims(g, 0, wchunks, steps, ntiles);
+    const size_t last = ((size_t)(wchunks - 1) * steps + (steps - 1)) * ntiles + (ntiles - 1);
+    return mc_rr_bank_bytes(g, 0) + (last * 64 + 63) * 16 + 16;
   }
   if (mc_is16(g.dtype)) {
     int chunks, steps, ntiles;
@@ -358,21 +457,28 @@
 int mc_pack_weights_batched(const mc_conv_desc* descs, const float* const* w_unique, const int32_t* dgrad,
                             void* const* packed, int32_t n, void* stream) {
   if (!descs || !w_unique || !dgrad || !packed || n <= 0) return MC_EINVAL;
-  for (int base = 0; base < n; base += PK_MAX) {
-    PkTable t;
-    t.n = n - base < PK_MAX ? n - base : PK_MAX;
-    int blocks = 0;
-    for (int k = 0; k < t.n; ++k) {
-      ConvGeom g;
-      int rc = geom_for(&descs[base + k], g);
-      if (rc) return rc;
-      if (!w_unique[base + k] || !packed[base + k]) return MC_EINVAL;
-      PkJob& j = t.j[k];
+  PkTable t;
+  t.n = 0;
+  int blocks = 0;
+  auto flush = [&]() {
+    if (t.n == 0) return;
+    hipLaunchKernelGGL(k_pack_batched, dim3(blocks), dim3(256), 0, (hipStream_t)stream, t);
+    t.n = 0; blocks = 0;
+  };
+  for (int k = 0; k < n; ++k) {
+    ConvGeom g;
+    int rc = geom_for(&descs[k], g);
+    if (rc) return rc;
+    if (!w_unique[k] || !packed[k]) return MC_EINVAL;
+    const bool rr = bank_is_rr(g, dgrad[k]);
+    for (int region = 0; region < ((rr && bank_has_tail(g, dgrad[k])) ? 2 : 1); ++region) {
+      if (t.n == PK_MAX) flush();
+      PkJob& j = t.j[t.n++];
       j.K = g.K; j.Cout = g.Cout; j.CBin = g.CBin; j.CB0 = g.CB0; j.Cin0 = g.Cin0; j.Cin1 = g.Cin1; j.Cin = g.Cin; j.U = g.U;
       j.nh = g.nh; j.nv = g.nv; j.nq = g.nq;
-      j.CBout = g.CBout; j.CinP = g.CinP; j.CoutP = g.CoutP; j.dgrad = dgrad[base + k]; j.bf16 = mc_is16(g.dtype);
+      j.CBout = g.CBout; j.CinP = g.CinP; j.CoutP = g.CoutP; j.dgrad = dgrad[k]; j.bf16 = mc_is16(g.dtype);
       j.f16 = (g.dtype == MC_MIX16 && !j.dgrad) ? 1 : 0;
-      j.rr = bank_is_rr(g, j.dgrad);
+      j.rr = rr && region == 0;
       size_t total;
       if (j.rr) {
         j.steps = 0;
@@ -387,15 +493,15 @@
         total = (size_t)(j.dgrad ? g.CBout : g.CBin) * g.K * g.K * 8 * (j.dgrad ? g.CinP : g.CoutP);
       }
       j.total = (unsigned)total;
-      j.w = w_unique[base + k];
-      j.out = packed[base + k];
+      j.w = w_unique[k];
+      j.out = (char*)packed[k] + (region ? mc_rr_bank_bytes(g, j.dgrad) : 0);
       j.first_block = blocks;
       int b = (int)((total + 256 * 8 - 1) / (256 * 8));
       blocks += b < 1 ? 1 : b;
     }
-    hipLaunchKernelGGL(k_pack_batched, dim3(blocks), dim3(256), 0, (hipStream_t)stream, t);
-    MC_CHECK_LAUNCH();
-  }
+  }
+  flush();
+  MC_CHECK_LAUNCH();
   return MC_OK;
 }
 
diff --git a/pbml_mantle_convection_amd/csrc/conv_bf16.hip b/pbml_mantle_convection_amd/csrc/conv_bf16.hip
--- a/pbml_mantle_convection_amd/csrc/conv_bf16.hip
+++ b/pbml_mantle_convection_amd/csrc/conv_bf16.hip
@@ -82,6 +82,14 @@
   const int my_items = (items - bid + (int)gridDim.x - 1) / (int)gridDim.x;
   const int total_stages = my_items * chunks;
 
+  if (FUSE == 0 && g.zslots > 0 && blockIdx.y == 0) {
+    const int per = g.zslots * g.CoutP * 2, zt = g.N * per;
+    for (int i = blockIdx.x * NTHR + threadIdx.x; i < zt; i += gridDim.x * NTHR) {
+      const int n = i / per;
+      fz.epart[((size_t)n * fz.estride + g.zslot0) * g.CoutP * 2 + (i - n * per)] = 0.f;
+    }
+  }
+
   constexpr int PER_CB = (TIH * TIW + NTHR - 1) / NTHR;
   static_assert(IN_ITERS <= CHUNK_CB * PER_CB, "");
   v4u rin[CHUNK_CB][PER_CB];
@@ -105,7 +113,8 @@
     const int jitem = t / chunks, ck = t - jitem * chunks;
     const int wi = bid + jitem * (int)gridDim.x;
     const int n = wi / g.tiles, tile = wi - n * g.tiles;
-    const int ty0 = (tile / g.tiles_x) * TH, tx0 = (tile % g.tiles_x) * TW;
+    int ty0, tx0, ye, xe;
+    conv_tile_rect(g, tile, TH, TW, ty0, tx0, ye, xe);
     const bool interior = (ty0 - g.pad >= 0) && (ty0 - g.pad + TIH <= g.H) && (tx0 - g.pad >= 0) && (tx0 - g.pad + TIW <= g.W);
     const unsigned org16 = (unsigned)((ty0 - g.pad) * g.W + (tx0 - g.pad)) * 16u;
 #pragma unroll
@@ -312,7 +321,8 @@
 
     const int wi = bid + jitem * (int)gridDim.x;
     const int n = wi / g.tiles, tile = wi - n * g.tiles;
-    const int ty0 = (tile / g.tiles_x) * TH, tx0 = (tile % g.tiles_x) * TW;
+    int ty0, tx0, ye, xe;
+    conv_tile_rect(g, tile, TH, TW, ty0, tx0, ye, xe);
     f32x2 s1[NTW][2], s2[NTW][2];
 #pragma unroll
     for (int tt = 0; tt < NTW; ++tt)
@@ -338,7 +348,7 @@
 #pragma unroll
       for (int i = 0; i < MT; ++i) {
         const int oy = oy0 + i / MTILES_X, ox = ox0 + (i % MTILES_X) * 16;
-        const bool inb = FULL || (oy < g.Ho && ox < g.Wo);
+        const bool inb = FULL || (oy < ye && ox < xe);
         const size_t off = (size_t)(i / MTILES_X) * row_bytes + (size_t)(i % MTILES_X) * 16 * 8 * (OUT_F32 ? 4 : 2);
 #pragma unroll
         for (int tt = 0; tt < NTW; ++tt) {
@@ -392,7 +402,7 @@
 #pragma unroll
         for (int i = 0; i < MT; ++i) {
           const int oy = oy0 + i / MTILES_X, ox = ox0 + (i % MTILES_X) * 16;
-          const bool inb = oy < g.Ho && ox < g.Wo;
+          const bool inb = oy < ye && ox < xe;
           const size_t off = (size_t)(i / MTILES_X) * row_bytes + (size_t)(i % MTILES_X) * 16 * 8 * 2;
           float yf[4];
           if constexpr (H16) {
@@ -426,7 +436,7 @@
       }
     };
     if constexpr (FUSE == 2) emit_dz();
-    else { if (ty0 + TH <= g.Ho && tx0 + TW <= g.Wo) emit(std::true_type{}); else emit(std::false_type{}); }
+    else { if (ty0 + TH <= ye && tx0 + TW <= xe) emit(std::true_type{}); else emit(std::false_type{}); }
     STAMP(5);
     if (FUSE == 2) part = fz.epart;
     if (part) {
@@ -450,7 +460,7 @@
           float r = 0.f;
 #pragma unroll
           for (int wv = 0; wv < WAVES / WN; ++wv) r += red[wv * WN + (int)(threadIdx.x >> 5) / NTW][threadIdx.x];
-          part[(((size_t)n * (FUSE == 2 ? fz.estride : g.tiles) + tile) * g.CoutP + co) * 2 + (threadIdx.x & 1)] = r;
+          part[(((size_t)n * (FUSE == 2 ? fz.estride : g.slots) + tile) * g.CoutP + co) * 2 + (threadIdx.x & 1)] = r;
         }
       }
     }
@@ -819,11 +829,11 @@
 #ifndef MC_NT1_MT
 #define MC_NT1_MT 8
 #endif
-inline Bf16Cfg cfg_for(int c_out, int k, int ho) {
+inline Bf16Cfg cfg_for(int c_out, int k, int ho, bool tail = false) {
   static const int th12 = getenv("MC_CONV_TH12") ? atoi(getenv("MC_CONV_TH12")) : 1;
   int ntiles = (c_out + 15) / 16;
   int nt = pick_nt(ntiles);
-  if (nt == 1) return {16, 32, 1, MC_NT1_MT};
+  if (nt == 1) return tail ? Bf16Cfg{16, 16, 1, 4} : Bf16Cfg{16, 32, 1, MC_NT1_MT};
   const bool t12 = th12 && k == 5 && (ho + 11) / 12 * 12 < (ho + 15) / 16 * 16;
   static const int th8 = getenv("MC_CONV_TH8") ? atoi(getenv("MC_CONV_TH8")) : 40;
   if (th8 && k == 5 && ho <= th8) return nt == 2 ? Bf16Cfg{8, 16, 2, 2} : Bf16Cfg{8, 16, 4, 2};
@@ -835,8 +845,8 @@
 
 }
 
-int mc_bf16_tile(const mc_conv_desc* d, int* th, int* tw) {
-  Bf16Cfg c = cfg_for(d->c_out, d->k, d->h + 2 * d->pad - d->k + 1);
+int mc_bf16_tile(const mc_conv_desc* d, bool tail, int* th, int* tw) {
+  Bf16Cfg c = cfg_for(d->c_out, d->k, d->h + 2 * d->pad - d->k + 1, tail);
   *th = c.th; *tw = c.tw;
   return MC_OK;
 }
@@ -882,7 +892,7 @@
 int mc_conv2d_bf16(const ConvGeom& g_in, const void* x0, const void* x1, const void* bank, const float* bias, void* y0,
                    void* y1, float* part, const ConvFuse& fz, int fuse, hipStream_t s) {
   const ConvGeom& g = g_in;
-  Bf16Cfg c = cfg_for(g.Cout, g.K, g.Ho);
+  Bf16Cfg c = cfg_for(g.Cout, g.K, g.Ho, g.tail != 0);
   int nt_total = (g.Cout + 15) / 16;
   int groups = (nt_total + c.nt - 1) / c.nt;
   int items = g.tiles * g.N;
@@ -907,13 +917,13 @@
   if (g.out_f32) {
     if (g.K == 5) LAUNCH(5, 16, 32, 1, MC_NT1_MT, true); else if (g.K == 3) LAUNCH(3, 16, 32, 1, MC_NT1_MT, true); else return MC_EUNSUPPORTED;
   } else if (g.K == 5) {
-    if (c.nt == 1) LAUNCH(5, 16, 32, 1, MC_NT1_MT, false);
+    if (c.nt == 1) { if (c.tw == 16) LAUNCH(5, 16, 16, 1, 4, false); else LAUNCH(5, 16, 32, 1, MC_NT1_MT, false); }
     else if (c.th == 24) LAUNCH_W(5, 24, 16, 4, 6, false, 1);
     else if (c.th == 12) { if (c.nt == 2) LAUNCH(5, 12, 16, 2, 3, false); else LAUNCH4(5, 12, 16, 3); }
     else if (c.th == 8) { if (c.nt == 2) LAUNCH(5, 8, 16, 2, 2, false); else LAUNCH4(5, 8, 16, 2); }
     else if (c.nt == 2) LAUNCH(5, 16, 16, 2, 4, false); else LAUNCH4(5, 16, 16, 4);
   } else if (g.K == 3) {
-    if (c.nt == 1) LAUNCH(3, 16, 32, 1, MC_NT1_MT, false); else if (c.nt == 2) LAUNCH(3, 16, 16, 2, 4, false); else LAUNCH4(3, 16, 16, 4);
+    if (c.nt == 1) { if (c.tw == 16) LAUNCH(3, 16, 16, 1, 4, false); else LAUNCH(3, 16, 32, 1, MC_NT1_MT, false); } else if (c.nt == 2) LAUNCH(3, 16, 16, 2, 4, false); else LAUNCH4(3, 16, 16, 4);
   } else {
     return MC_EUNSUPPORTED;
   }
diff --git a/pbml_mantle_convection_amd/csrc/conv_common.h b/pbml_mantle_convection_amd/csrc/conv_common.h
--- a/pbml_mantle_convection_amd/csrc/conv_common.h
+++ b/pbml_mantle_convection_amd/csrc/conv_common.h
@@ -14,6 +14,11 @@
   int nh, nv, nq;
   int dtype;
   int out_f32;
+  int oy0, ox0, oye, oxe, tiles_a;
+  int by0, bx0, bye, bxe, tiles_xb;
+  int slots;
+  int zslot0, zslots;
+  int tail;
 };
 
 struct ConvFuse {
@@ -81,6 +86,9 @@
   g.tiles_x = (g.Wo + tile_w - 1) / tile_w;
   g.tiles_y = (g.Ho + tile_h - 1) / tile_h;
   g.tiles = g.tiles_x * g.tiles_y;
+  g.oy0 = g.ox0 = 0; g.oye = g.Ho; g.oxe = g.Wo; g.tiles_a = g.tiles;
+  g.by0 = g.bx0 = g.bye = g.bxe = 0; g.tiles_xb = 1;
+  g.slots = g.tiles; g.zslot0 = g.zslots = 0; g.tail = 0;
   g.sym_h = d->sym_h; g.nh = d->sym_h / 2; g.nv = d->sym_v / 2; g.nq = d->sym_hv / 4;
   g.U = d->c_out - g.nh - g.nv - 3 * g.nq;
   g.dtype = d->dtype;
@@ -107,6 +115,16 @@
   if (G > work) G = work;
   g.wgrad_G = (int)G;
   return MC_OK;
+}
+
+__device__ __forceinline__ void conv_tile_rect(const ConvGeom& g, int tile, int th, int tw, int& ty0, int& tx0, int& ye, int& xe) {
+  const bool b = tile >= g.tiles_a;
+  const int t = b ? tile - g.tiles_a : tile, nx = b ? g.tiles_xb : g.tiles_x;
+  const int r = t / nx;
+  ty0 = (b ? g.by0 : g.oy0) + r * th;
+  tx0 = (b ? g.bx0 : g.ox0) + (t - r * nx) * tw;
+  ye = b ? g.bye : g.oye;
+  xe = b ? g.bxe : g.oxe;
 }
 
 static __host__ __device__ inline int cin_padded_index(int ci, int Cin0, int CB0) {
diff --git a/pbml_mantle_convection_amd/csrc/conv_rr_bf16.hip b/pbml_mantle_convection_amd/csrc/conv_rr_bf16.hip
--- a/pbml_mantle_convection_amd/csrc/conv_rr_bf16.hip
+++ b/pbml_mantle_convection_amd/csrc/conv_rr_bf16.hip
@@ -681,6 +681,10 @@
                  float* part, const ConvFuse& fz, int fuse, hipStream_t s) {
   if (g.K != 5 && g.K != 3) return MC_EUNSUPPORTED;
   if (fuse == 2 && g.out_f32) return MC_EUNSUPPORTED;
+  if (g.oy0 != 0 || g.ox0 != 0 || g.tiles_a != g.tiles || (g.oye != g.Ho && g.oye % RR_R) || (g.oxe != g.Wo && g.oxe % RR_TW) ||
+      g.tiles_y != (g.oye + RR_R - 1) / RR_R || g.tiles_x != (g.oxe + RR_TW - 1) / RR_TW || g.tiles != g.tiles_x * g.tiles_y ||
+      (part && g.slots != g.tiles * RR_STRIPS))
+    return MC_EINVAL;
   const bool gelu = fuse == 2 ? fz.eact == MC_ACT_GELU
                               : ((fz.act0 == MC_ACT_GELU || (fz.act0 == MC_ACT_NONE && !fz.coef0)) &&
                                  (fz.act1 == MC_ACT_GELU || (fz.act1 == MC_ACT_NONE && !fz.coef1)));
```

Measured after the change: 3158 samples/s (median of 2 runs). 1.1% lower.
